# BlueFisher/Advanced-Soft-Actor-Critic

Measured on AMD Instinct MI355X. Metric: SAC train steps/sec (PER sample + grad step), batch 256, higher is better.
Workload: dtype f32; 1 GPU; cfg2: TEST vector obs(6) c_action(2) stock MLP, PER capacity 524288, n_step=4 V-trace; per_gpu_batch=256, global_batch=256, rows_resident=262144, replay_capacity=524288, n_step=4, burn_in_step=0, parallelism=single, ranks=1, hipgraph=True

## Files before the change

advanced-soft-actor-critic_amd/algorithm/fused_mlp.py:

```python
import weakref

import torch
from torch import nn

from asac_amd import native

from .nn_models.layers.linear_layers import LinearLayers, ResBlock
from .param_grads import (SUM_PARTIALS_LATER, DeferredPartialSums, direct_enabled, direct_param_grads,
                          direct_skips, flat_alias)

__all__ = ['StockMLP', 'describe_q', 'describe_policy', 'describe_dense', 'fused_dense', 'gauss_head']

MAX_WIDTH, MAX_HEAD = 64, 16
MAX_INPUT = 128
FUSED_DENSE = True


def _blocks_of(ll: LinearLayers):
    blocks, final = [], None
    for m in ll.dense:
        if isinstance(m, ResBlock):
            if final is not None or not isinstance(m.act, nn.GELU) or getattr(m.act, 'approximate', 'none') != 'none':
                return None
            blocks.append(m)
# ... 242 lines not shown
        x0, x1 = ctx.saved_tensors
        x1 = x1 if ctx.has_x1 else None
        need0, need1 = ctx.needs_input_grad[1], ctx.has_x1 and ctx.needs_input_grad[2]
        g0, g1, pg = _backward_delivering(ctx, x0, x1, grad_out, need0, need1)
        return (None, g0, g1, None, None, *pg)


class _MlpSelectFn(torch.autograd.Function):

    @staticmethod
    def forward(ctx, anchor, base, t, x1, mlp, param_grads, *params):
        x0 = base[:, t]
        out = mlp._launch_forward(x0, x1)
        ctx.mlp, ctx.param_grads, ctx.t, ctx.n_params = mlp, param_grads, t, len(params)
        ctx.save_for_backward(base, x1 if x1 is not None else base.new_empty(0))
        ctx.has_x1 = x1 is not None
        return out

    @staticmethod
    def backward(ctx, grad_out):
        base, x1 = ctx.saved_tensors
        x1 = x1 if ctx.has_x1 else None
        mlp, t = ctx.mlp, ctx.t
        need0, need1 = ctx.needs_input_grad[1], ctx.has_x1 and ctx.needs_input_grad[3]
        g0, g1, pg = _backward_delivering(ctx, base[:, t], x1, grad_out, need0, need1, reduce_members=False)
        g_base = None
        if g0 is not None:
            key = (tuple(base.shape), t % base.shape[1], base.device)
            g_base = mlp._window_grads.get(key)
            if g_base is None:
                if len(mlp._window_grads) > 4:
                    mlp._window_grads.clear()
                g_base = mlp._window_grads[key] = torch.zeros_like(base)
            torch.sum(g0, dim=0, out=g_base[:, t])
        if g1 is not None and x1.dim() == 2:
            g1 = g1.sum(0) if mlp.E > 1 else g1[0]
        return (None, g_base, None, g1, None, None, *pg)


class StockMLP:

    def __init__(self, desc, flat, grad_flat, start, member_stride, E, device, param_tensors=()):
        self.desc, self.E, self.member_stride = desc, E, member_stride
        self._window_grads = {}
        self.wide = desc.in0 + desc.in1 > MAX_WIDTH
        self.param_tensors = list(param_tensors)
        self.params = flat[start:start + E * member_stride]
        self.grad_params = None if grad_flat is None else grad_flat[start:start + E * member_stride]
        self.in0, self.in1 = desc.in0, desc.in1
        self.out_cols = desc.head_cols[0] + desc.head_cols[1]
        self._anchor = torch.zeros(1, device=device, requires_grad=True)
        self.accumulate = True
        self._workspace = None
        self._start, self._deferred_rows = start, None
        self.device = device

    @staticmethod
    def _rows(x, width):
        assert x.shape[-1] == width
        if x.dim() == 2 and x.stride(-1) == 1:
            return x
        return x.reshape(-1, width) if x.is_contiguous() else x.contiguous().view(-1, width)

    @staticmethod
    def _rows_in_place(x, width):
        assert x.shape[-1] == width
        if x.dim() == 3 and not x.is_contiguous() and x.stride(2) == 1 and x.stride(0) != x.stride(1) * x.shape[1]:
            return native.WindowRows(x)
        return StockMLP._rows(x, width)

    def _launch_forward(self, x0, x1, out=None):
        job, out = self.job(x0, x1, out)
        if isinstance(x0, native.WindowRows):
            native.mlp_forward_multi([job])
        else:
            native.mlp_forward(job)
        return out

    def _workspace_for(self, N):
        need = native.mlp_backward_workspace(self.member_stride, self.E, N)
        if self._workspace is None or self._workspace.numel() < need:
            self._workspace = torch.zeros(need, dtype=torch.float32, device=self.device)
        return self._workspace

    def _reduce_mode(self, defer):
        if defer:
            return native.MLP_REDUCE_DEFER
        return native.MLP_REDUCE_ACCUMULATE if self.accumulate else native.MLP_REDUCE_OVERWRITE

    def backward_qloss(self, x0, x1, target_q, y, weights, clip_eps, loss_out, defer=False, state_grads=False):
        N = x0.shape[-2]
        g0 = torch.empty((self.E, N, self.in0), dtype=torch.float32, device=self.device) if state_grads else None
        native.mlp_backward_qloss(self._pass(x0, x1), target_q, y, weights, clip_eps, loss_out, self.grad_params,
                                  self._workspace_for(N), self._reduce_mode(defer), grad_x0=g0)
        self._deferred_rows = N if defer else None
        return g0

    def backward_qloss_return_ok(self, N: int, ret) -> bool:
        return native.mlp_backward_qloss_return_ok(self._pass(None, None, N=N), ret)

    def backward_qloss_return(self, x0, x1, target_q, ret, weights, clip_eps, loss_out, defer=False, state_grads=False):
        N = x0.shape[-2]
        g0 = torch.empty((self.E, N, self.in0), dtype=torch.float32, device=self.device) if state_grads else None
        native.mlp_backward_qloss_return(self._pass(x0, x1), target_q, ret, weights, clip_eps, loss_out, self.grad_params,
                                         self._workspace_for(N), self._reduce_mode(defer), grad_x0=g0)
        self._deferred_rows = N if defer else None
        return g0

    def backward_policy_q(self, x0, x1, q_table, subset, E_sample):
        N = x0.shape[-2]
        g1 = torch.empty((self.E, N, self.in1), dtype=torch.float32, device=self.device)
        native.mlp_backward_policy_q(self._pass(x0, x1), q_table, subset, E_sample, g1)
        return g1

    def backward_policy_sample(self, x0, eps, grad_a, log_alpha, defer=False, offline=None):
        N = x0.shape[-2]
        native.mlp_backward_policy_sample(self._pass(x0, None), eps, grad_a, log_alpha, self.grad_params,
                                          self._workspace_for(N), self._reduce_mode(defer), offline=offline)
        self._deferred_rows = N if defer else None

    def policy_step_fused_ok(self, critics: 'StockMLP', N: int) -> bool:
        return (self.E == 1 and critics.E >= 2 and self.grad_params is not None and
                native.policy_step_fused_ok(critics.desc, critics.params, critics.member_stride, self.desc, self.params,
                                            self.member_stride, N))

    def policy_step_fused(self, critics: 'StockMLP', x0, action, eps, log_alpha, q_out=None, defer=False, subset=None,
                          sample_out=None, offline=None):
        N = x0.shape[-2]
        assert subset is not None or critics.E == 2
        a_out, logp_out, ls_out = sample_out if action is None else (None, None, None)
        native.policy_step_fused(critics.desc, critics.params, critics.member_stride, self.desc, self.params,
                                 self.member_stride, x0, N, action, eps, log_alpha, q_out, self.grad_params,
                                 self._workspace_for(N), self._reduce_mode(defer), subset=subset, a_out=a_out,
                                 logp_out=logp_out, ls_out=ls_out, offline=offline)
        self._deferred_rows = N if defer else None

    def adam_partials(self, opt, loss_out=None):
        N = self._deferred_rows
        assert N is not None, 'no deferred backward pending'
        tiles = native.mlp_backward_tiles(N, self.E)
        s0 = self._start
        s1 = s0 + self.E * self.member_stride
        native.adam_step_partials(self.params, self.grad_params, opt.exp_avg[s0:s1], opt.exp_avg_sq[s0:s1], opt.lr,
                                  opt.betas[0], opt.betas[1], opt.eps, opt.steps_done, self._workspace, tiles,
                                  self.E, self.member_stride, native.mlp_param_extent(self.desc),
                                  self.accumulate, loss_out, N if loss_out is not None else 0)
        self._deferred_rows = None

    def _pass(self, x0, x1, out=None, N=None) -> 'native.MlpJob':
        if N is None:
            N = x0.shape[0] if isinstance(x0, native.WindowRows) else x0.shape[-2]
        return native.mlp_job(self.desc, self.params, self.member_stride, self.E, x0, x1, N, out)

    def job(self, x0, x1, out=None):
        N = x0.shape[0] if isinstance(x0, native.WindowRows) else x0.shape[-2]
        if self.wide and isinstance(x0, native.WindowRows):
            x0 = x0.t.reshape(N, x0.t.shape[-1])
        if out is None:
            out = torch.empty((self.E, N, self.out_cols), dtype=torch.float32, device=self.device)
        assert out.shape == (self.E, N, self.out_cols) and out.is_contiguous()
        return self._pass(x0, x1, out), out

    def _launch_backward(self, x0, x1, grad_out, need0, need1, param_grads, reduce_members=True, defer=False,
                         grad_target=None, later=None):
        N = x0.shape[-2]
        E = self.E
        g0 = torch.empty((E, N, self.in0), dtype=torch.float32, device=self.device) if need0 else None
        g1 = torch.empty((E, N, self.in1), dtype=torch.float32, device=self.device) if need1 else None
        gp = ws = None
        mode = self._reduce_mode(defer and param_grads)
        if param_grads:
            gp = self.grad_params
            self._deferred_rows = N if defer else None
            if grad_target is not None:
                assert not defer
                gp, mode = grad_target, native.MLP_REDUCE_OVERWRITE
            if later is None or defer:
                ws = self._workspace_for(N)
            if later is not None and not defer:
                ws = torch.empty(native.mlp_backward_workspace(self.member_stride, E, N), dtype=torch.float32,
                                 device=self.device)
                tiles, used = native.mlp_backward_tiles(N, E), native.mlp_param_extent(self.desc)
                for e in range(E):
                    later.add(ws[e * self.member_stride:], tiles, 16 if tiles >= 64 else 1, E * self.member_stride, used,
                              gp[e * self.member_stride:], accumulate=mode == native.MLP_REDUCE_ACCUMULATE)
                mode = native.MLP_REDUCE_DEFER
        native.mlp_backward(self._pass(x0, x1), grad_out, g0, g1, gp, ws, reduce_mode=mode)
# ... 46 lines not shown
```

advanced-soft-actor-critic_amd/algorithm/sac_base.py:

```python
import contextlib
import logging
import random
from collections import defaultdict, namedtuple
from pathlib import Path

import numpy as np
import torch
from torch import distributions, nn
from torch.nn import functional

from asac_amd import native

from . import fused_gru, fused_linear
from .fused import DeviceNoise, FlatAdam, FlatParamGroup, squash_sample, squash_sample_ls, time_slice
from .fused_mlp import StockMLP, describe_policy, describe_q
from .nn_models import *
from .nn_models.layers.seq_layers import step_mask_cache
from .nn_models.representation import ModelSimpleRep
from .normalizer import Normalizer, fused_normalizer_applies
from .param_grads import direct_param_grads, learner_backward
from .batch_buffer import BatchBuffer
from .captured_step import CapturedStep
from .replay_buffer import PrioritizedReplayBuffer
from .sac_aux import AuxHeadsMixin
# ... 201 lines not shown
        self.ensemble_q_sample = ensemble_q_sample
        self.burn_in_step = burn_in_step
        self.n_step = n_step
        self.seq_encoder = seq_encoder
        self.write_summary_per_step = int(write_summary_per_step)
        self.save_model_per_step = int(save_model_per_step)
        self.batch_size = batch_size
        self.tau = tau
        self.update_target_per_step = update_target_per_step
        self.use_auto_alpha = use_auto_alpha
        self.target_d_alpha = target_d_alpha
        self.target_c_alpha = target_c_alpha
        self.d_policy_entropy_penalty = d_policy_entropy_penalty
        self.learning_rate = learning_rate
        self.gamma = gamma
        self.v_lambda = v_lambda
        self.v_rho = v_rho
        self.v_c = v_c
        self.clip_epsilon = clip_epsilon
        self.discrete_dqn_like = discrete_dqn_like
        self.discrete_dqn_epsilon = discrete_dqn_epsilon
        self.use_n_step_is = use_n_step_is
        self.siamese = siamese
        self.siamese_use_q = siamese_use_q
        self.siamese_use_adaptive = siamese_use_adaptive
        self.use_prediction = use_prediction
        self.transition_kl = transition_kl
        self.use_extra_data = use_extra_data
        self.curiosity = curiosity
        self.curiosity_strength = curiosity_strength
        self.use_rnd = use_rnd
        self.rnd_n_sample = rnd_n_sample
        self.use_normalization = use_normalization
        self.offline_enabled = offline_enabled
        self.offline_loss = offline_loss
        self.action_noise = action_noise

        hip_config = dict(hip_config or {})
        self._use_graph = bool(hip_config.get('use_graph', True))
        self._graph_warmup = int(hip_config.get('graph_warmup', 3))
        self._direct_graph_launch = bool(hip_config.get('direct_graph_launch', True))
        self._dist = hip_config.get('dist')
        self._use_fused_mlp = bool(hip_config.get('fused_mlp', True))
        self._graph_collectives = bool(hip_config.get('graph_collectives', True))
        self._twin_rep = bool(hip_config.get('twin_rep', True))
        self._fuse_linear_tanh = bool(hip_config.get('fused_linear_tanh', True))
        self._use_sidecars = bool(hip_config.get('sidecars', True))
        self._defer_is_weights = bool(hip_config.get('defer_is_weights', True))
        self._fused_policy_step = bool(hip_config.get('fused_policy_step', True))
        self._fused_forward_chain = bool(hip_config.get('fused_forward_chain', True))
        self._fused_td_chain = bool(hip_config.get('fused_td_chain', True))
        self._fused_td_update = bool(hip_config.get('fused_td_update', True))
        self._fused_q_return = bool(hip_config.get('fused_q_return', True))
        self._fused_q_state_grads = bool(hip_config.get('fused_q_state_grads', True))
        self._gru_backward_at = bool(hip_config.get('gru_backward_at', True))
        self._adjacent_cat = bool(hip_config.get('adjacent_cat', True))
        self._fold_rep_q_adam = bool(hip_config.get('fold_rep_q_adam', True))
        self._rep_grad_one_position = bool(hip_config.get('rep_grad_one_position', True))
        self._deferred_cat = bool(hip_config.get('deferred_cat', True))
        self._rep_from_burn_in = bool(hip_config.get('rep_from_burn_in', True))
        self._fused_curiosity = bool(hip_config.get('fused_curiosity', True))
        self._fused_discrete = bool(hip_config.get('fused_discrete', True))
        self._fused_dqn = bool(hip_config.get('fused_dqn', True))
        self._fused_rnd = bool(hip_config.get('fused_rnd', True))
        self._fused_offline = bool(hip_config.get('fused_offline', True))
        self._rnd_stacks = None
        self._rnd_buffers = {}
        self._fused_rnd_discrete = bool(hip_config.get('fused_rnd_discrete', True))
        self._drnd_stacks = None
        self._drnd_buffers = {}
        self._fused_act = bool(hip_config.get('fused_act', True))
        self._fused_siamese = bool(hip_config.get('fused_siamese', False))
        self._fused_hybrid = bool(hip_config.get('fused_hybrid', False))
        self._fused_normalizer = bool(hip_config.get('fused_normalizer', False))
        self.normalizer = None
        self._siamese_ws = {}
        self._fused_rpm_loss = bool(hip_config.get('fused_rpm_loss', True))
        self._rpm_single_backward = bool(hip_config.get('rpm_single_backward', True))
        self._fused_gating = bool(hip_config.get('fused_gating', True))
        self._rpm_conv_one_launch = bool(hip_config.get('rpm_conv_one_launch', True))
        self._lookahead = int(hip_config.get('lookahead', 0))
        assert self._lookahead in (0, 1), 'hip_config lookahead: 0 (synchronous sampling) or 1 (one batch in flight)'
        self._la_gather_sidecar = bool(hip_config.get('lookahead_gather_sidecar', True)) and self._use_sidecars
        self._head_gather_sidecar = bool(hip_config.get('head_gather_sidecar', True)) and self._use_sidecars
        self._head_gather = None
        self._head_gather_w = False
        self._head_plan_cache = None
        self._la_gather = None
        self._fuse_prediction_dense = bool(hip_config.get('fuse_prediction_dense', True))
        self._fused_q_loss_with_aux = bool(hip_config.get('fused_q_loss_with_aux', True))
        self._head_sums_members = bool(hip_config.get('head_sums_members', True))
        self._rep_epilogue, self._rep_epilogue_hp = False, None
        self._cat_mode = None
        self._g_state_base = None
        self._dist_sampling = hip_config.get('dist_sampling', 'throughput')
        self._dist_ready = False
        assert self._dist_sampling in ('throughput', 'parity')

        self._set_logger()

        if not use_replay_buffer:
            if self._dist is not None:
                raise ValueError('use_replay_buffer=False (the episode batch queue) is single-GPU: a data-parallel '
                                 "context (hip_config['dist']) is not supported with it")
            if self._lookahead:
                self._logger.info("hip_config['lookahead'] does not apply without a replay buffer: forced to 0")
# ... 161 lines not shown
        self._fq = self._ftq = self._fpi = None
        if self._use_fused_mlp and self.c_action_size and not self.d_action_sizes:
            dq = [describe_q(q) for q in self.model_q_list + self.model_target_q_list]
            seg = self._params.segments
            stride = seg['q_0'][1] - seg['q_0'][0]
            consecutive = all(seg[f'q_{i}'][0] == seg['q_0'][0] + i * stride for i in range(self.ensemble_q_num))
            if all(d is not None for d in dq) and consecutive:
                tseg = self._target_params.segments
                self._fq = StockMLP(dq[0], self._params.flat, self._params.grad, seg['q_0'][0], stride,
                                    self.ensemble_q_num, dev, [p for q in self.model_q_list for p in q.parameters()])
                self._ftq = StockMLP(dq[0], self._target_params.flat, None, tseg['q_0'][0], stride,
                                     self.ensemble_q_num, dev)
            dp = describe_policy(self.model_policy)
            if dp is not None:
                self._fpi = StockMLP(dp, self._params.flat, self._params.grad, seg['policy'][0],
                                     seg['policy'][1] - seg['policy'][0], 1, dev, list(self.model_policy.parameters()))
        self._wide_critics = self._fq is not None and self._fq.wide
        if self._wide_critics:
            self._la_gather_sidecar = False
        self._logger.info(f'fused stock MLP path: Q={self._fq is not None} policy={self._fpi is not None}')
        stock_only = {f'q_{i}' for i in range(self.ensemble_q_num)} | {'policy', 'alpha'}
        self._grads_overwrite = (self._fq is not None and self._fpi is not None and not self.offline_enabled
                                 and all(stop == start or name in stock_only
                                         for name, (start, stop) in self._params.segments.items()))
        if self._grads_overwrite:
            self._fq.accumulate = self._fpi.accumulate = False

        n, A, E, Es = self.n_step, self.c_action_size, self.ensemble_q_num, self.ensemble_q_sample
        f32 = dict(dtype=torch.float32, device=dev)
        A1 = max(A, 1)
        sizes = [B * (n + 1) * A1, B * A1, B * A1, B * (n + 1) * A1]
        self._eps_all = torch.zeros(sum(sizes), **f32)
        o = np.cumsum([0] + sizes)
        self._eps_y = self._eps_all[o[0]:o[1]].view(B, n + 1, A1)
        self._eps_pi = self._eps_all[o[1]:o[2]].view(B, A1)
        self._eps_alpha = self._eps_all[o[2]:o[3]].view(B, A1)
        self._eps_td = self._eps_all[o[3]:o[4]].view(B, n + 1, A1)
        names = ('y_dn', 'y_dnext', 'y_cn', 'y_cnext', 'pi_d', 'pi_c', 'td_dn', 'td_dnext', 'td_cn', 'td_cnext')
        self._subsets_all = torch.arange(Es, dtype=torch.int32, device=dev).repeat(len(names), 1).contiguous()
        self._subsets = {k: self._subsets_all[i] for i, k in enumerate(names)}
        self._y_buf = torch.zeros(B, **f32)
        self._y_td_buf = torch.zeros(B, **f32)
        self._td_error = torch.zeros(B, **f32)
        self._stats = {k: torch.zeros((), **f32) for k in ('d_entropy', 'c_entropy', 'loss_curiosity', 'loss_policy')}
        self._loss_q_e = torch.zeros(E, **f32)
        self._stats['loss_q'] = self._loss_q_e[0]
        self._grad_q = torch.zeros(E, B, **f32)
        self._mse_big_ws = torch.zeros(native.mse_mean_grad_workspace(), **f32) if self.use_prediction else None
        self._grad_logp = torch.zeros(B, **f32)
        self._branches = native.branches(self.d_action_sizes) if self.d_action_sizes else None
        self._discrete_grads = {}
        self._hybrid_bufs = {}
        self._ls_y = None
        self._cq_buf, self._tq_buf, self._cq_td_buf = (torch.zeros(E, B, 1, **f32) for _ in range(3))
        self._pi_q, self._pi_stats_src = torch.zeros(E, B, 1, **f32), None
        self._pi_a, self._pi_logp, self._pi_sampled = torch.zeros(B, A1, **f32), torch.zeros(B, **f32), False
        self._rep_twin = None
        if self._twin_rep and type(self.model_rep) is not ModelSimpleRep:
            from .fused_gru import TwinPass
            self._rep_twin = TwinPass(self.model_rep, self.model_target_rep)

    def _build_ckpt(self) -> None:
        ck = self.ckpt_dict = {'global_step': self.global_step}
        if self.optimizer_rep is not None:
            ck['model_rep'], ck['model_target_rep'], ck['optimizer_rep'] = \
                self.model_rep, self.model_target_rep, self.optimizer_rep
        for i in range(self.ensemble_q_num):
            ck[f'model_q_{i}'] = self.model_q_list[i]
            ck[f'model_target_q_{i}'] = self.model_target_q_list[i]
            ck[f'optimizer_q_{i}'] = self.optimizer_q_list[i]
        ck['model_policy'], ck['optimizer_policy'] = self.model_policy, self.optimizer_policy
        ck['log_d_alpha'], ck['log_c_alpha'] = self.log_d_alpha, self.log_c_alpha
        if self.use_auto_alpha:
            ck['optimizer_alpha'] = self.optimizer_alpha
        if self.curiosity == CURIOSITY.FORWARD:
            ck['model_forward_dynamic'] = self.model_forward_dynamic
        elif self.curiosity == CURIOSITY.INVERSE:
            ck['model_inverse_dynamic'] = self.model_inverse_dynamic
        if self.curiosity is not None:
            ck['optimizer_curiosity'] = self.optimizer_curiosity
        self._aux_ckpt(ck)
        total = sum(p.numel() for m in ck.values() if isinstance(m, nn.Module) for p in m.parameters())
        self._logger.info(f'Parameters: {total}')

    def _init_or_restore(self, last_ckpt: int | None) -> None:
        self.ckpt_dir = None
        if not self.model_abs_dir:
            self._update_target_variables()
            return
        self.ckpt_dir = ckpt_dir = Path(self.model_abs_dir).joinpath('model')
        ckpts = sorted(int(p.stem) for p in ckpt_dir.glob('*.pth')) if ckpt_dir.exists() else []
        ckpt_dir.mkdir(parents=True, exist_ok=True)
        if not ckpts:
            self._logger.info('Initializing from scratch')
            self._update_target_variables()
            return
        if last_ckpt is None or last_ckpt not in ckpts:
            if last_ckpt is not None:
                self._logger.warning(f'{last_ckpt} NOT IN {ckpts}, using {ckpts[-1]}')
            last_ckpt = ckpts[-1]
        path = ckpt_dir.joinpath(f'{last_ckpt}.pth')
        restored = torch.load(path, map_location=self.device, weights_only=True)
        failed = False
        for name, obj in self.ckpt_dict.items():
            if name not in restored:
                self._logger.warning(f'{name} not in {last_ckpt}.pth')
# ... 761 lines not shown
            if d_q_online is not None:
                args.td_error_out = td_out.data_ptr()
            native.discrete_return(args, self._branches, [q[0] for q in nx_qs], d_logits, action=nx_actions,
                                   q_online=d_q_online)
            d_y = y_out.unsqueeze(-1)
        elif self.d_action_sizes:
            sub_next, sub_n = self._subsets[subset_prefix + '_dnext'], self._subsets[subset_prefix + '_dn']
            self.noise.subset_(sub_next, E)
            self.noise.subset_(sub_n, E)
            stacked = torch.stack([q[0] for q in nx_qs])
            mean_next = stacked[:, :, 1:].index_select(0, sub_next.long()).mean(0)
            mean_n = stacked[:, :, :-1].index_select(0, sub_n.long()).mean(0)
            probs = d_policy.probs
            n_p, next_p = probs[:, :-1], probs[:, 1:]
            d_alpha = torch.exp(self.log_d_alpha)
            v_n = torch.sum(n_p * (mean_n - d_alpha * torch.log(n_p.clamp(min=1e-8))), -1) / self.d_action_branch_size
            v_next = torch.sum(next_p * (mean_next - d_alpha * torch.log(next_p.clamp(min=1e-8))), -1) \
                / self.d_action_branch_size
            pi, mu = self._stored_action_ratios(d_policy, n_mu_probs, nx_actions) if self.use_n_step_is else (None, None)
            d_y = torch.empty(n_rewards.shape[0], dtype=torch.float32, device=self.device)
            args = self._vtrace_args(n_rewards, n_dones, n_last_masks, n_padding_masks, d_y)
            native.vtrace_return_direct(args, v_n.contiguous(), v_next.contiguous(), pi, mu)
            d_y = d_y.unsqueeze(-1)

        if self.c_action_size:
            sub_n, sub_next = self._subsets[subset_prefix + '_cn'], self._subsets[subset_prefix + '_cnext']
            self.noise.subset_(sub_n, E)
            self.noise.subset_(sub_next, E)
            if q_table is not None:
                q_tab = q_table
            elif nx_qs is not None:
                q_tab = torch.stack([q[1] for q in nx_qs]).squeeze(-1)
            else:
                q_tab = self._c_q_values(True, nx_states, a_tanh, nx_obses_list)
            ret = self._c_return(q_tab, logp, c_pi, n_mu_probs, sub_n, sub_next, n_rewards, n_dones, n_last_masks,
                                 n_padding_masks, y_out, q_online, td_out)
            if launch:
                self._launch_return(ret)
            c_y = y_out.unsqueeze(-1)
        return (d_y, c_y) if launch else (d_y, c_y, ret)

    def _stock_q_targets(self, job_tq, job_pi, ls, window, policy_sample):
        nx_states, nx_actions = window[3], window[4]
        ls = ls[0].view(*nx_states.shape[:2], 2 * self.c_action_size)
        pre = self._return_sample_epilogue([job_tq, job_pi], 1, ls, nx_actions, self._eps_y, policy_sample)
        if pre is None:
            native.mlp_forward_multi([job_tq, job_pi])
        sample, stored_pi = pre or (None, None)
        _, c_y, ret = self._get_y(*window, eps_buf=self._eps_y, subset_prefix='y', y_out=self._y_buf, ls=ls,
                                  sample=sample, stored_pi=stored_pi, policy_sample=policy_sample and pre is None,
                                  launch=False)
        return c_y, ret

    def _stock_q_backward(self, x0, a0, ret, c_y, priority_is, fold, fused_return, state_grads=False):
        w = priority_is.reshape(-1).contiguous() if priority_is is not None else None
        t_q = self._tq_buf.view(self.ensemble_q_num, -1)
        if fused_return and self._fq.backward_qloss_return_ok(x0.shape[-2], ret.args):
            g0 = self._fq.backward_qloss_return(x0, a0, t_q, ret.args, w, self.clip_epsilon, self._loss_q_e,
                                                defer=fold, state_grads=state_grads)
        else:
            self._launch_return(ret)
            g0 = self._fq.backward_qloss(x0, a0, t_q, c_y.reshape(-1), w, self.clip_epsilon, self._loss_q_e,
                                         defer=fold, state_grads=state_grads)
        if fold:
            self._fq.adam_partials(self.optimizer_q_list[0], loss_out=self._loss_q_e)
        return g0

    @torch.no_grad()
    def _train_rep_q_stock(self, n_last_masks, n_padding_masks, nx_obses_list, nx_states, nx_actions, n_rewards,
                           n_dones, n_mu_probs, priority_is, policy_sample):
        E, B = self.ensemble_q_num, nx_states.shape[0]
        x0 = StockMLP._rows(nx_states[:, 0], self.state_size)
        a0 = StockMLP._rows(nx_actions[:, 0], self.c_action_size)
        xs = StockMLP._rows(nx_states, self.state_size)
        job_tq, _ = self._ftq.job(x0, a0, out=self._tq_buf)
        job_pi, ls = self._fpi.job(xs, None)
        T, A = nx_states.shape[1], self.c_action_size
        window = (n_last_masks, n_padding_masks, nx_obses_list, nx_states, nx_actions, n_rewards, n_dones,
                  n_mu_probs if self.use_n_step_is else None)
        fused = None
        if self._fused_forward_chain and self.curiosity is None:
            f32 = dict(dtype=torch.float32, device=self.device)
            a_y, logp_y = torch.empty((B, T, A), **f32), torch.empty((B, T), **f32)
            c_pi = torch.empty((B, T, A), **f32) if self.use_n_step_is else None
            job_q, q_tab = self._ftq.job(xs, a_y.view(-1, A))
            fused = native.pi_q_job(job_pi, job_q, self._eps_y, a_y, logp_y, T,
                                    action=nx_actions if self.use_n_step_is else None,
                                    action_offset=self.d_action_summed_size, prob_out=c_pi,
                                    eps2=self._eps_pi if policy_sample else None, t2=0,
                                    a2_out=self._pi_a, logp2_out=self._pi_logp)
            if not native.policy_sample_q_forward_ok(fused):
                fused = None
        riders = None
        if fused is not None and self._head_gather is not None:
            ring = self._head_ring_job(fused, job_tq, self._head_gather, nx_states, nx_actions)
            if ring is not None:
                fused, riders = ring, [self._head_gather['sidecar_w' if self._head_gather_w else 'sidecar']]
                self._head_gather = None
        self._join_head_gather()
        if fused is not None:
            self.noise.normal_(self._eps_y)
            if policy_sample:
                self.noise.normal_(self._eps_pi)
                self._pi_sampled = True
            native.policy_sample_q_forward(fused, [job_tq], sidecars=riders if riders is not None else self._take_la_gather())
            _, c_y, ret = self._get_y(*window, eps_buf=self._eps_y, subset_prefix='y', y_out=self._y_buf,
                                      ls=ls[0].view(B, T, 2 * A), sample=(a_y, logp_y), stored_pi=c_pi,
                                      q_table=q_tab.view(E, B, T), launch=False)
        else:
            c_y, ret = self._stock_q_targets(job_tq, job_pi, ls, window, policy_sample)
        opt = self.optimizer_q_list[0]
        fold = self._dist is None and opt.start == self._fq._start and self._params.span('rep')[0] == self._params.span('rep')[1]
        self._stock_q_backward(x0, a0, ret, c_y, priority_is, fold, fused_return=fused is not None and self._fused_q_return)
        if not fold:
            self._finish_rep_q(None, None)

    def _head_ring_job(self, fused, job_tq, head, nx_states, nx_actions):
        rb, b = self.replay_buffer, self.burn_in_step
        obs, act = rb._batch[f'obs_{self.obs_names[0]}'], rb._batch['action']
        if b != rb.prev_n or nx_states.shape[1] + b != rb.window:
            return None
        for view, whole in ((nx_states, obs), (nx_actions, act)):
            at = whole[:, b:]
            if view.data_ptr() != at.data_ptr() or view.stride() != at.stride() or view.shape != at.shape:
                return None
        job = native.pi_q_ring_rows(fused, rb._ids, head['index_ring'], rb.capacity, rb.prev_n, rb.window, b, head['x0'],
                                    head['action'], x_j0=b, x_action_offset=self.d_action_summed_size)
        return job if native.policy_sample_q_forward_ok(job, [job_tq]) else None

    def _train_rep_q(self, n_last_masks, n_padding_masks, nx_obses_list, nx_states, nx_actions, n_rewards,
                     n_dones, n_mu_probs, priority_is, aux=None, policy_sample=False, state_base=None):
        if (self._stock_c_only() and aux is None and self.clip_epsilon > 0 and not nx_states.requires_grad
                and self.optimizer_rep is None):
            return self._train_rep_q_stock(n_last_masks, n_padding_masks, nx_obses_list, nx_states, nx_actions,
                                           n_rewards, n_dones, n_mu_probs, priority_is, policy_sample)
        self._join_head_gather()
        dsum = self.d_action_summed_size
        obs_list = [o[:, 0] for o in nx_obses_list]
        state, action = nx_states[:, 0], nx_actions[:, 0]
        if state_base is not None and not nx_states.requires_grad:
            state = state_base[0][:, state_base[1]]
        d_action, c_action = action[..., :dsum], action[..., dsum:]

        if (self._fused_q_state_grads and self._fq is not None and self._ftq is not None and self._fpi is not None
                and not self.d_action_sizes
                and self.c_action_size and self.clip_epsilon > 0 and aux is None and state_base is not None
                and state_base[0].dim() == 3 and state.requires_grad):
            base, t = state_base
            with torch.no_grad():
                x0 = StockMLP._rows(base.detach()[:, t], self.state_size)
                a0 = StockMLP._rows(c_action, self.c_action_size)
                states_y = nx_states.detach()
                job_tq, _ = self._ftq.job(x0, a0, out=self._tq_buf)
                job_pi, ls_y = self._fpi.job(StockMLP._rows_in_place(states_y, self.state_size), None)
                c_y, ret = self._stock_q_targets(
                    job_tq, job_pi, ls_y, (n_last_masks, n_padding_masks, nx_obses_list, states_y, nx_actions, n_rewards,
                                           n_dones, n_mu_probs if self.use_n_step_is else None), policy_sample)
                fold = self._dist is None and self._fold_rep_q_adam and self._rep_q_adam_alike()
                g0 = self._stock_q_backward(x0, a0, ret, c_y, priority_is, fold, fused_return=self._fused_q_return,
                                            state_grads=True)
                g_base = self._g_state_base
                if g_base is None or g_base.shape != base.shape:
                    g_base = self._g_state_base = torch.zeros_like(base)
                at_position = self._gru_backward_at and fused_gru.is_fused_top(base)
                from_head = not at_position and self._head_sums_members and fused_linear.is_fused_head_output(base)
                if not (at_position or from_head):
# ... 110 lines not shown
    def _finish_rep_q(self, total_loss, loss_q0, aux=None, ctx=None):
        if total_loss is not None:
            with learner_backward():
                total_loss.backward(retain_graph=aux is not None and self.use_prediction)
            self._stats['loss_q'].copy_(loss_q0.detach())
        start, stop = self._params.span('rep', f'q_{self.ensemble_q_num - 1}')
        if aux is None:
            if self._dist is not None:
                self._dist.all_reduce_grads(self._params.grad, start, stop)
            self.optimizer_q_list[0].step(start, stop)
            return
        grads_rep_main = [p.grad.detach() for p in self.model_rep.parameters()]
        grads_q_main = [[p.grad.detach() for p in q.parameters()] for q in self.model_q_list]
        if self.siamese is not None:
            n_obs = [o[:, :-1] for o in ctx['nx_obses_list']]
            self._train_siamese_representation_learning(grads_rep_main, grads_q_main, aux['n_indexes'],
                                                        ctx['n_padding_masks'], n_obs, aux['n_pre_actions'],
                                                        aux['n_pre_seq_hidden_states'])
        q_start = self._params.span('q_0')[0]
        if self._dist is not None:
            self._dist.all_reduce_grads(self._params.grad, q_start, stop)
        self.optimizer_q_list[0].step(q_start, stop)
        if self.use_prediction:
            self._train_rpm(grads_rep_main, ctx['nx_obses_list'], ctx['nx_states'], aux['nx_target_states'],
                            ctx['nx_actions'][:, :-1], ctx['n_rewards'])
        if self.optimizer_rep is not None:
            if self._dist is not None:
                self._dist.all_reduce_grads(self._params.grad, *self._params.span('rep'))
            self.optimizer_rep.step()

    def _stock_c_only(self) -> bool:
        return (self._fpi is not None and self._fq is not None and bool(self.c_action_size)
                and not self.d_action_sizes and (not (self.offline_enabled and self.offline_loss) or self._offline_fused()))

    def _offline_fused(self) -> bool:
        return fused_offline_applies(
            enabled=self._fused_offline, plain_learner=type(self)._plain_learner,
            offline_loss=self.offline_enabled and self.offline_loss, c_action_size=self.c_action_size,
            d_action_sizes=self.d_action_sizes, stock_networks=self._fq is not None and self._fpi is not None,
            data_parallel=self._dist is not None,
            float32_on_device=self._params.flat.dtype == torch.float32 and self._params.flat.is_cuda)

    def _offline_plain(self) -> bool:
        return bool(self._fused_offline and type(self)._plain_learner and self._dist is None
                    and self._params.flat.dtype == torch.float32 and self._params.flat.is_cuda)

    @torch.no_grad()
    def _train_policy_stock(self, state, ls=None, offline=None):
        A, E = self.c_action_size, self.ensemble_q_num
        x = StockMLP._rows(state, self.state_size)
        B = x.shape[0]
        fusable = (self._fused_policy_step and self.ensemble_q_sample == 2 and self._fpi.policy_step_fused_ok(self._fq, B))
        sample_out = None
        if ls is None and not self._pi_sampled and fusable:
            f32 = dict(dtype=torch.float32, device=self.device)
            self.noise.normal_(self._eps_pi)
            sample_out = (torch.empty((B, A), **f32), torch.empty(B, **f32), torch.empty((B, 2 * A), **f32))
            a_tanh, logp, scale = sample_out[0], sample_out[1], sample_out[2][:, A:]
        else:
            if ls is None:
                ls = self._fpi._launch_forward(x, None)[0]
            loc, scale = ls[..., :A], ls[..., A:]
            if self._pi_sampled:
                a_tanh, logp, self._pi_sampled = self._pi_a, self._pi_logp, False
            else:
                self.noise.normal_(self._eps_pi)
                a_tanh = torch.empty((B, A), dtype=torch.float32, device=self.device)
                logp = torch.empty(B, dtype=torch.float32, device=self.device)
                native.squash_sample_fwd(loc, scale, self._eps_pi, a_tanh, logp)
        sub = self._subsets['pi_c']
        self.noise.subset_(sub, E)
        self._pi_stats_src = (logp, scale) if offline is None else (
            logp, scale, sample_out[2] if sample_out is not None else ls, self._eps_pi, offline)
        opt = self.optimizer_policy
        fold = self._dist is None and (opt.start, opt.stop) == (self._fpi._start, self._fpi._start + self._fpi.member_stride)
        if fusable and a_tanh.is_contiguous():
            self._fpi.policy_step_fused(self._fq, x, None if sample_out is not None else a_tanh, self._eps_pi,
                                        self.log_c_alpha, q_out=self._pi_q, defer=fold, subset=sub if E != 2 else None,
                                        sample_out=sample_out, offline=offline)
        else:
            c_qs = self._fq._launch_forward(x, a_tanh, out=self._pi_q)
            g_a = self._fq.backward_policy_q(x, a_tanh, c_qs.view(E, B), sub if self.ensemble_q_sample != E else None,
                                             self.ensemble_q_sample)
            self._fpi.backward_policy_sample(x, self._eps_pi, g_a, self.log_c_alpha, defer=fold, offline=offline)
        if fold:
            self._fpi.adam_partials(opt)
            return
        if self._dist is not None:
            self._dist.all_reduce_grads(self._params.grad, *self._params.span('policy'))
        opt.step()

    def _train_policy(self, obs_list, state, action, mu_d_policy_probs, ls=None):
        dsum, E = self.d_action_summed_size, self.ensemble_q_num
        offline = self.offline_enabled and self.offline_loss
        if self._stock_c_only():
            return self._train_policy_stock(state, ls, offline=action[..., dsum:] if offline else None)
        if self._discrete_fused(state.shape[0]):
            logits = self._discrete_logits(state, obs_list)
            with torch.no_grad():
                d_qs = [q(state, action[..., dsum:], obs_list)[0] for q in self.model_q_list]
            sub = self._subsets['pi_d']
            self.noise.subset_(sub, E)
            _, grad_logits = self._discrete_grad_buffers(state.shape[0])
            native.discrete_policy_loss_grad(self._branches, logits.detach(), d_qs, sub, self.ensemble_q_sample,
                                             mu_d_policy_probs, self.log_d_alpha, self.d_policy_entropy_penalty,
                                             self._stats['loss_policy'], grad_logits, self._stats['d_entropy'])
            pi_inputs = list(self.model_policy.parameters())
            with direct_param_grads(only=pi_inputs):
                torch.autograd.backward([logits], [grad_logits], inputs=pi_inputs)
            self.optimizer_policy.step()
            return
        if self._hybrid_fused(state.shape[0]):
            logits, loc, scale = self._hybrid_heads(state, obs_list)
            with torch.no_grad():
                d_qs = [q(state, action[..., dsum:], obs_list)[0] for q in self.model_q_list]
            sub_d = self._subsets['pi_d']
            self.noise.subset_(sub_d, E)
            self.noise.normal_(self._eps_pi)
            a_tanh, logp = squash_sample(loc, scale, self._eps_pi)
            c_qs = torch.stack([q(state, a_tanh, obs_list)[1] for q in self.model_q_list]).squeeze(-1)
            sub_c = self._subsets['pi_c']
            self.noise.subset_(sub_c, E)
            buf = self._hybrid_buffers(state.shape[0])
            native.hybrid_policy_loss_grad(
                self._branches, logits.detach(), d_qs, sub_d, mu_d_policy_probs, self.log_d_alpha,
                self.d_policy_entropy_penalty, logp.detach(), c_qs.detach().contiguous(),
                sub_c if self.ensemble_q_sample != E else None, self.ensemble_q_sample, self.log_c_alpha, scale.detach(),
                self._stats['loss_policy'], buf['grad_logits'], buf['grad_logp'], buf['grad_cq'], self._stats['d_entropy'],
                self._stats['c_entropy'])
# ... 860 lines not shown
```

advanced-soft-actor-critic_amd/csrc/mlp.hip:

```cpp
#include "asac_common.h"
#include "asac_gelu.h"
#include "asac_sidecar.h"
#include "asac_squash.h"
#include "asac_vtrace.h"

#include <cmath>

namespace asac {

constexpr int kP = 66;
constexpr int kMaxW = 64;
constexpr int kMaxB = ASAC_MLP_MAX_BLOCKS;
constexpr int kHeadPad = 16;
#ifndef ASAC_PS_WAVES
#define ASAC_PS_WAVES 16
#endif
#ifndef ASAC_PIQ_WAVES
#define ASAC_PIQ_WAVES 8
#endif
constexpr int kPiQThreads = 64 * ASAC_PIQ_WAVES;
template <int TM> constexpr int threads_of() { return TM * 16; }

inline int mlp_tile_rows(int64_t N, int E) { return ((N + 15) / 16) * (int64_t)(E > 0 ? E : 1) <= 256 ? 16 : 32; }

using f32x4 = __attribute__((ext_vector_type(4))) float;

#ifdef ASAC_MLP_STAMPS
__device__ unsigned long long g_mlp_stamps[32];
#define MLP_STAMP(i)                                                                             \
    do {                                                                                         \
        if (blockIdx.x == 0 && blockIdx.y == 0 && threadIdx.x == 0) g_mlp_stamps[i] = wall_clock64(); \
    } while (0)
#define MLP_STAMP_AT(i, t)                                                                       \
    do {                                                                                         \
        if (blockIdx.x == 0 && blockIdx.y == 0 && threadIdx.x == (t)) g_mlp_stamps[i] = wall_clock64(); \
    } while (0)
#else
#define MLP_STAMP(i)
#define MLP_STAMP_AT(i, t)
#endif

__device__ __forceinline__ void lds_barrier() {
    __builtin_amdgcn_fence(__ATOMIC_RELEASE, "workgroup", "local");
    __builtin_amdgcn_s_barrier();
    __builtin_amdgcn_fence(__ATOMIC_ACQUIRE, "workgroup", "local");
}

__device__ __forceinline__ void loads_landed() { __builtin_amdgcn_s_waitcnt(0x0F70); }

__device__ __forceinline__ int round4(int v) { return (v + 3) & ~3; }

template <int THREADS>
__device__ __forceinline__ void stage_matrix(float* dst, const float* __restrict__ src, int rows, int cols) {
    if (rows == kMaxW && cols == kMaxW && (reinterpret_cast<uintptr_t>(src) & 15) == 0) {
        constexpr int U = 1024 / THREADS;
        const float4* s4 = reinterpret_cast<const float4*>(src);
        float4 v[U];
#pragma unroll
        for (int u = 0; u < U; ++u) v[u] = s4[threadIdx.x + u * THREADS];
// ... 779 lines not shown
    s += __shfl_xor(s, 16, 64);
    s += __shfl_xor(s, 32, 64);
    if (lane < 16 && c < J) out[c] = s;
}

__device__ __forceinline__ void grad_weight_tiles(const float* __restrict__ delta, int jbase, const float* __restrict__ xprev,
                                                  int J, int K, float* __restrict__ out, int worker, int workers) {
    if (worker < 0) return;
    const int lane = threadIdx.x & 63;
    const int lr = lane & 15, lk = lane >> 4;
    const int njt = (J + 15) >> 4, nkt = (K + 15) >> 4;
    const bool vec = (K & 3) == 0 && (reinterpret_cast<uintptr_t>(out) & 15) == 0;
    for (int t = worker; t < njt * nkt; t += workers) {
        const int jt = t / nkt, kt = t - jt * nkt;
        float dv[4], xv[4];
#pragma unroll
        for (int i = 0; i < 4; ++i) {
            dv[i] = delta[(4 * i + lk) * kP + jbase + jt * 16 + lr];
            xv[i] = xprev[(4 * i + lk) * kP + kt * 16 + lr];
        }
        __builtin_amdgcn_sched_barrier(0);
        f32x4 acc0 = {0.f, 0.f, 0.f, 0.f}, acc1 = {0.f, 0.f, 0.f, 0.f};
        acc0 = __builtin_amdgcn_mfma_f32_16x16x4f32(xv[0], dv[0], acc0, 0, 0, 0);
        acc1 = __builtin_amdgcn_mfma_f32_16x16x4f32(xv[1], dv[1], acc1, 0, 0, 0);
        acc0 = __builtin_amdgcn_mfma_f32_16x16x4f32(xv[2], dv[2], acc0, 0, 0, 0);
        acc1 = __builtin_amdgcn_mfma_f32_16x16x4f32(xv[3], dv[3], acc1, 0, 0, 0);
        const f32x4 acc = acc0 + acc1;
        const int j = jt * 16 + lr, k0 = kt * 16 + 4 * lk;
        if (j >= J) continue;
        float* o = out + j * K + k0;
        if (vec && k0 + 3 < K) {
            *reinterpret_cast<float4*>(o) = make_float4(acc[0], acc[1], acc[2], acc[3]);
        } else {
#pragma unroll
            for (int r = 0; r < 4; ++r)
                if (k0 + r < K) o[r] = acc[r];
        }
    }
}
template <int NW = ASAC_PS_WAVES>
__device__ __forceinline__ void ps_grad_weight(const float* __restrict__ delta, int jbase, const float* __restrict__ xprev,
                                               int J, int K, float* __restrict__ out, int first_wave = 0) {
    grad_weight_tiles(delta, jbase, xprev, J, K, out, ((threadIdx.x >> 6) + NW - first_wave) & (NW - 1), NW);
}

template <bool RET>
struct RetIn {};
template <>
struct RetIn<true> {
    asac_vtrace_args_t v;
    int32_t seg;
};

template <int TM, bool WIDE, int NB, bool RET = false, int W8 = 0>
__global__ __launch_bounds__(W8 ? 64 * W8 : TM * 16) void k_mlp_bwd(const MlpArgs a, const RetIn<RET> rv) {
    static_assert(W8 == 0 || ((W8 == 8 || W8 == 16) && TM == 16 && NB == 3 && !WIDE), "8 / 16 waves: 16-row tiles of the stock networks");
    constexpr int THREADS = W8 ? 64 * W8 : threads_of<TM>();
    constexpr int RT = TM / 16;
    constexpr bool fixed = NB > 0;
    static_assert(!(fixed && WIDE), "the fixed-shape path has a first layer of <= 64 inputs");
    extern __shared__ __attribute__((aligned(16))) unsigned char smem_raw[];
    MlpBwdLds<TM>& L = *reinterpret_cast<MlpBwdLds<TM>*>(smem_raw);
    const int e = blockIdx.y;
    const int64_t row0 = (int64_t)blockIdx.x * TM;
    const float* P = a.params + e * a.member_stride;
    float* part = a.partial ? a.partial + ((int64_t)blockIdx.x * gridDim.y + e) * a.member_stride : nullptr;
    const int wave = threadIdx.x >> 6, lane = threadIdx.x & 63;
    const bool comp = !W8 || wave < 4;
    const int rt = wave % RT, ct = comp ? wave / RT : 0;
    const int nb = fixed ? NB : a.d.n_blocks;
    const int K0 = a.d.in0 + a.d.in1;
    const int O = a.d.head_cols[0] + a.d.head_cols[1];
    const int col = ct * 16 + (lane & 15);

    MLP_STAMP(0);
    [[maybe_unused]] float ql_tq[4] = {0.f, 0.f, 0.f, 0.f}, ql_w[4] = {1.f, 1.f, 1.f, 1.f}, ql_y[4] = {0.f, 0.f, 0.f, 0.f};
    constexpr bool wide = WIDE;
    float* x_hi = L.x[kMaxB];
    float* w_hi = L.w[nb < kMaxB ? nb : kMaxB - 1];
    if constexpr (fixed) {
        const StageScalars q = stage_scalars<NB>(a, e);
        constexpr int SLOTS = TM * 64 / THREADS;
        float in_lo[SLOTS];
        fetch_input_tile_fixed<THREADS, false, SLOTS>(q, e, row0, in_lo);
        const int r = threadIdx.x >> 4, c = threadIdx.x & 15;
        const int64_t row = row0 + r;
        float gin = 0.f;
        if (a.gout && r < TM) {
            const float t = a.gout[((int64_t)e * a.N + (row < a.N ? row : a.N - 1)) * O + (c < O ? c : O - 1)];
            gin = (row < a.N && c < O) ? t : 0.f;
        }
        StagedNet<THREADS> regs;
        net_fetch_fixed<THREADS, NB>(q, regs);
        if constexpr (W8 != 0) {
            if (!a.gout && !a.eps && !a.q_table && wave < RT) {
#pragma unroll
                for (int rr = 0; rr < 4; ++rr) {
                    const int64_t lr_row = row0 + wave * 16 + 4 * (lane >> 4) + rr;
                    const int64_t rc = lr_row < a.N ? lr_row : a.N - 1;
                    ql_tq[rr] = a.tq[(int64_t)e * a.N + rc];
                    if (a.w) ql_w[rr] = a.w[rc];
                    if constexpr (!RET) ql_y[rr] = a.y[rc];
                }
            }
        }
        if constexpr (RET) {
            const asac_vtrace_args_t& v = rv.v;
            const int n = v.n, pitch = (n + 1) | 1;
            float* s_d = reinterpret_cast<float*>(smem_raw + sizeof(MlpBwdLds<TM>));
            float* s_c = s_d + TM * pitch;
            float* s_v0 = s_c + TM * pitch;
            const int f = threadIdx.x, fr = f / n, ft = f - fr * n;
            const bool have = f < TM * n && row0 + fr < a.N;
            VtraceStepRaw raw{};
// ... 267 lines not shown
    if (comp && (a.gx0 || a.gx1)) {
#pragma unroll
        for (int r = 0; r < 4; ++r) {
            const int64_t row = row0 + rt * 16 + 4 * (lane >> 4) + r;
            if (row >= a.N) continue;
            if (col < a.d.in0) {
                if (a.gx0) a.gx0[((int64_t)e * a.N + row) * a.d.in0 + col] = g[r];
            } else if (col < K0) {
                if (a.gx1) a.gx1[((int64_t)e * a.N + row) * a.d.in1 + (col - a.d.in0)] = g[r];
            }
            const int ch = col + kMaxW;
            if (wide && ch < K0) {
                if (ch < a.d.in0) {
                    if (a.gx0) a.gx0[((int64_t)e * a.N + row) * a.d.in0 + ch] = g_hi[r];
                } else if (a.gx1) {
                    a.gx1[((int64_t)e * a.N + row) * a.d.in1 + (ch - a.d.in0)] = g_hi[r];
                }
            }
        }
    }
    MLP_STAMP(10);
}

constexpr int kPsWaves = ASAC_PS_WAVES;
constexpr int kPsThreads = 64 * kPsWaves;
constexpr int kPsSlots = 1024 / kPsThreads;
constexpr int kPsRows = 16;

struct PsQLds {
    float w[3][kMaxW * kP];
    float head[kHeadPad * kP];
    float bias[3][kMaxW];
    float head_bias[kHeadPad];
    float xs[2][kPsRows * kP];
};
struct PsPiLds {
    float w[3][kMaxW * kP];
    float head[kHeadPad * kP];
    float bias[3][kMaxW];
    float head_bias[kHeadPad];
    float x[4][kPsRows * kP];
    float delta[kPsRows * kP];
    float delta2[kPsRows * kP];
};
struct PsLds {
    PsQLds q[2];
    float ga[2][kPsRows * kHeadPad];
    float qv[2][kPsRows];
    float ls[kPsRows * 2 * kHeadPad];
    float act[kPsRows * kHeadPad];
};
static_assert(sizeof(PsPiLds) <= 2 * sizeof(PsQLds), "the policy phase reuses the critics' LDS");

struct PolicyStepArgs {
    MlpArgs q, pi;
    float* q_out;
    float* a_out;
    float* logp_out;
    float* ls_out;
};

__device__ __forceinline__ void ps_fetch_tile(const StageScalars& q, int64_t row0, float (&v)[kPsSlots]) {
    const int in0 = q.in0, in1 = q.in1;
    const rsrc_t r0 = make_rsrc(q.x0);
    const rsrc_t r1 = make_rsrc(q.x1, in1 > 0 ? 0x7fffffffu : 0u);
#pragma unroll
    for (int u = 0; u < kPsSlots; ++u) {
        const int i = threadIdx.x + u * kPsThreads;
        const int r = i >> 6, c = i & 63;
        const uint32_t row = (uint32_t)row0 + (uint32_t)r;
        const bool live = (int64_t)row0 + r < q.N;
        const unsigned o0 = (live && c < in0) ? (row * (uint32_t)q.x0_rs + (uint32_t)c) * 4u : kOob;
        const unsigned o1 = (live && c >= in0 && c < in0 + in1) ? (row * (uint32_t)q.x1_rs + (uint32_t)(c - in0)) * 4u : kOob;
        v[u] = __builtin_bit_cast(float, buf_ld(r0, o0) | buf_ld(r1, o1));
    }
}
__device__ __forceinline__ void ps_put_tile(const float (&v)[kPsSlots], float* xs) {
#pragma unroll
    for (int u = 0; u < kPsSlots; ++u) {
        const int i = threadIdx.x + u * kPsThreads;
        xs[(i >> 6) * kP + (i & 63)] = v[u];
    }
}

template <bool OFFLINE>
__global__ __launch_bounds__(kPsThreads) void k_policy_step(const PolicyStepArgs a_by_value) {
    extern __shared__ __attribute__((aligned(16))) unsigned char smem_raw[];
    const ASAC_KARG PolicyStepArgs& a = *static_cast<const ASAC_KARG PolicyStepArgs*>(kernarg_base());
    PsLds& L = *reinterpret_cast<PsLds*>(smem_raw);
    PsPiLds& P = *reinterpret_cast<PsPiLds*>(smem_raw);
    const int wave = threadIdx.x >> 6, lane = threadIdx.x & 63;
    const int m = wave >> 2, ct = wave & 3;
    const int col = ct * 16 + (lane & 15);
    const int64_t row0 = (int64_t)blockIdx.x * kPsRows;
    const int64_t N = a.pi.N;
    const int A = a.pi.d.head_cols[0];
    const int S = a.q.d.in0, K0q = a.q.d.in0 + a.q.d.in1, K0p = a.pi.d.in0;
    MLP_STAMP(0);

    const int e0 = a.q.subset ? a.q.subset[0] : 0, e1 = a.q.subset ? a.q.subset[1] : 1;
    const StageScalars s0 = stage_scalars<3>(a.q, e0), s1 = stage_scalars<3>(a.q, e1), sp = stage_scalars<3>(a.pi, 0);
    const bool sample_here = a.q.x1 == nullptr;
    float in_q[kPsSlots] = {}, in_pi[kPsSlots];
    if (!sample_here) ps_fetch_tile(s0, row0, in_q);
    ps_fetch_tile(sp, row0, in_pi);
    StagedNet<kPsThreads> r0, r1, rp;
    net_fetch_fixed<kPsThreads, 3>(s0, r0);
    net_fetch_fixed<kPsThreads, 3>(s1, r1);
    net_fetch_fixed<kPsThreads, 3>(sp, rp);
    float ev = 0.f, gl = 0.f;
    {
        const int lrow = threadIdx.x / (A > 0 ? A : 1), d = threadIdx.x - lrow * A;
        if ((int)threadIdx.x < kPsRows * A && row0 + lrow < N) ev = a.pi.eps[(row0 + lrow) * A + d];
        gl = expf(*a.pi.log_alpha) * (1.f / (float)N);
    }
    [[maybe_unused]] float av = 0.f;
    if constexpr (OFFLINE) {
        const int lrow = threadIdx.x / (A > 0 ? A : 1), d = threadIdx.x - lrow * A;
        if ((int)threadIdx.x < kPsRows * A && row0 + lrow < N) av = a.pi.off_action[(row0 + lrow) * a.pi.off_row_stride + d];
    }
    if (sample_here) {
        net_put_fixed<kPsThreads, 3>(rp, P);
        ps_put_tile(in_pi, P.x[0]);
        __syncthreads();
#pragma unroll
        for (int l = 0; l < 3; ++l) {
            if (wave < 4) {
                const float* xin = P.x[l & 1];
                float* xout = P.x[(l & 1) ^ 1];
                const f32x4 acc = l > 0 ? gemm_tile(xin, P.w[l], kMaxW, 0, wave) : gemm_tile(xin, P.w[l], round4(K0p), 0, wave);
                const int pc = wave * 16 + (lane & 15);
                const float bias = P.bias[l][pc];
                const bool res = a.pi.d.residual[l] != 0;
                f32x2_g ya, yb, unused;
                gelu_parts2((f32x2_g){acc[0] + bias, acc[1] + bias}, ya, unused);
                gelu_parts2((f32x2_g){acc[2] + bias, acc[3] + bias}, yb, unused);
                const float yv[4] = {ya.x, ya.y, yb.x, yb.y};
#pragma unroll
                for (int r = 0; r < 4; ++r) {
                    const int row = 4 * (lane >> 4) + r;
                    float y = yv[r];
                    if (res) y += xin[row * kP + pc];
                    xout[row * kP + pc] = y;
                }
            }
            __syncthreads();
        }
        if (wave < 4) {
            const f32x4 acc = gemm_tile(P.x[1], P.head, kMaxW, 0, 0);
            const int hc = lane & 15;
            const float mine = wave == 0 ? acc[0] : wave == 1 ? acc[1] : wave == 2 ? acc[2] : acc[3];
            const int lrow = 4 * (lane >> 4) + wave;
            const float v = head_value(a.pi.d, hc, mine + P.head_bias[hc]);
            L.ls[lrow * 2 * kHeadPad + hc] = v;
            if (a.ls_out && row0 + lrow < N && hc < 2 * A) a.ls_out[(row0 + lrow) * (2 * A) + hc] = v;
        }
        __syncthreads();
        if (threadIdx.x < kPsRows) {
            const int lrow = threadIdx.x;
            const int64_t r = row0 + lrow;
            float* arow = L.act + lrow * kHeadPad;
            if (r < N) {
                float lp;
                squash_sample_at(L.ls + lrow * 2 * kHeadPad, L.ls + lrow * 2 * kHeadPad + A, a.pi.eps + r * A, A, arow, &lp, nullptr);
                for (int d = 0; d < A; ++d) a.a_out[r * A + d] = arow[d];
                a.logp_out[r] = lp;
            } else {
                for (int d = 0; d < A; ++d) arow[d] = 0.f;
            }
        }
        __syncthreads();
        ps_put_tile(in_pi, L.q[0].xs[0]);
        ps_put_tile(in_pi, L.q[1].xs[0]);
    } else {
        ps_put_tile(in_q, L.q[0].xs[0]);
        ps_put_tile(in_q, L.q[1].xs[0]);
    }
    net_put_fixed<kPsThreads, 3>(r0, L.q[0]);
    net_put_fixed<kPsThreads, 3>(r1, L.q[1]);
    __syncthreads();
    if (sample_here) {
        if ((int)threadIdx.x < kPsRows * A) {
            const int lrow = threadIdx.x / A, d = threadIdx.x - lrow * A;
            const float v = L.act[lrow * kHeadPad + d];
            L.q[0].xs[0][lrow * kP + S + d] = v;
            L.q[1].xs[0][lrow * kP + S + d] = v;
        }
        __syncthreads();
    }
    MLP_STAMP(1);

    const bool qwave = wave < 8;
    PsQLds& Q = L.q[qwave ? m : 0];
    f32x4 z[3];
    int cur = 0;
#pragma unroll
    for (int l = 0; l < 3; ++l) {
        if (qwave) {
        const float* xin = Q.xs[cur];
        float* xout = Q.xs[cur ^ 1];
        const f32x4 acc = l > 0 ? gemm_tile(xin, Q.w[l], kMaxW, 0, ct) : gemm_tile(xin, Q.w[l], round4(K0q), 0, ct);
        const float bias = Q.bias[l][col];
        const bool res = a.q.d.residual[l] != 0;
        f32x2_g ya, yb, da, db;
        gelu_parts2((f32x2_g){acc[0] + bias, acc[1] + bias}, ya, da);
        gelu_parts2((f32x2_g){acc[2] + bias, acc[3] + bias}, yb, db);
        const float yv[4] = {ya.x, ya.y, yb.x, yb.y};
        z[l] = f32x4{da.x, da.y, db.x, db.y};
#pragma unroll
        for (int r = 0; r < 4; ++r) {
            const int row = 4 * (lane >> 4) + r;
            float y = yv[r];
            if (res) y += xin[row * kP + col];
            xout[row * kP + col] = y;
        }
        }
        __syncthreads();
        cur ^= 1;
    }
    MLP_STAMP(2);
    if (qwave && ct == 0) {
        const f32x4 raw = gemm_tile(Q.xs[cur], Q.head, kMaxW, 0, 0);
        if ((lane & 15) == 0) {
#pragma unroll
            for (int r = 0; r < 4; ++r) {
                const int lrow = 4 * (lane >> 4) + r;
                const float qv = raw[r] + Q.head_bias[0];
                L.qv[m][lrow] = qv;
                if (a.q_out && row0 + lrow < N) a.q_out[(int64_t)(m ? e1 : e0) * N + row0 + lrow] = qv;
            }
        }
    }
    __syncthreads();
    MLP_STAMP(3);
    float* qdelta = Q.xs[cur ^ 1];
    if (qwave) {
        const int t = threadIdx.x & 255;
        const int r = t >> 4, c = t & 15;
        float g = 0.f;
        if (c == 0 && row0 + r < N) {
            const int best = L.qv[1][r] < L.qv[0][r] ? 1 : 0;
            if (best == m) g = -1.f / (float)N;
        }
        qdelta[r * kP + c] = g;
    }
    __syncthreads();
    MLP_STAMP(4);
    f32x4 g = {0.f, 0.f, 0.f, 0.f};
    if (qwave) g = gemm_tile_nt(qdelta, Q.head, kHeadPad, 0, ct);
#pragma unroll
    for (int l = 2; l >= 0; --l) {
        qdelta = Q.xs[cur ^ (l & 1)];
        if (qwave) {
#pragma unroll
            for (int r = 0; r < 4; ++r) qdelta[(4 * (lane >> 4) + r) * kP + col] = g[r] * z[l][r];
        }
        __syncthreads();
        if (qwave && (l > 0 || (ct * 16 < K0q && ct * 16 + 16 > S))) {
            f32x4 gin = gemm_tile_nt(qdelta, Q.w[l], kMaxW, 0, ct);
            if (a.q.d.residual[l]) gin += g;
            g = gin;
        }
    }
    if (qwave && col >= S && col < K0q) {
#pragma unroll
        for (int r = 0; r < 4; ++r) L.ga[m][(4 * (lane >> 4) + r) * kHeadPad + (col - S)] = g[r];
    }
    __syncthreads();
    MLP_STAMP(5);

    net_put_fixed<kPsThreads, 3>(rp, P);
    ps_put_tile(in_pi, P.x[0]);
    if (threadIdx.x < kPsRows * kHeadPad) P.delta[(threadIdx.x >> 4) * kP + (threadIdx.x & 15)] = 0.f;
    loads_landed();
    __syncthreads();
    MLP_STAMP(6);
    f32x4 zp[3];
#pragma unroll
    for (int l = 0; l < 3; ++l) {
        if (wave < 4) {
            const float* xin = P.x[l];
            float* xout = P.x[l + 1];
            const f32x4 acc = l > 0 ? gemm_tile(xin, P.w[l], kMaxW, 0, wave) : gemm_tile(xin, P.w[l], round4(K0p), 0, wave);
            const int pc = wave * 16 + (lane & 15);
            const float bias = P.bias[l][pc];
            const bool res = a.pi.d.residual[l] != 0;
            f32x2_g ya, yb, da, db;
            gelu_parts2((f32x2_g){acc[0] + bias, acc[1] + bias}, ya, da);
            gelu_parts2((f32x2_g){acc[2] + bias, acc[3] + bias}, yb, db);
            const float yv[4] = {ya.x, ya.y, yb.x, yb.y};
            zp[l] = f32x4{da.x, da.y, db.x, db.y};
#pragma unroll
            for (int r = 0; r < 4; ++r) {
                const int row = 4 * (lane >> 4) + r;
                float y = yv[r];
                if (res) y += xin[row * kP + pc];
                xout[row * kP + pc] = y;
            }
        }
        __syncthreads();
    }
    MLP_STAMP(7);
    if (wave == 0) {
        const f32x4 raw = gemm_tile(P.x[3], P.head, kMaxW, 0, 0);
        const int hc = lane & 15;
#pragma unroll
        for (int r = 0; r < 4; ++r) P.delta[(4 * (lane >> 4) + r) * kP + hc] = raw[r] + P.head_bias[hc];
    }
    __syncthreads();
    MLP_STAMP(8);
    if ((int)threadIdx.x < kPsRows * A) {
        const int lrow = threadIdx.x / A, d = threadIdx.x - lrow * A;
        const int64_t row = row0 + lrow;
        float g_loc = 0.f, g_scale = 0.f;
        const float raw_l = P.delta[lrow * kP + d], raw_s = P.delta[lrow * kP + A + d];
        if (row < N) {
            const float loc = head_value(a.pi.d, d, raw_l), sc = head_value(a.pi.d, A + d, raw_s);
            const float u = loc + ev * sc;
            const float t = tanhf(u);
            const float one_m = 1.f - t * t;
            float ga = 0.f;
            ga += L.ga[0][lrow * kHeadPad + d];
            ga += L.ga[1][lrow * kHeadPad + d];
            float gx = ga * one_m;
            if (one_m > 1e-2f) gx += gl * ((float)A * 2.f * t);
            if constexpr (OFFLINE) gx += offline_grad_u(u, av, 1.f / (float)N);
            g_loc = gx * head_deriv(a.pi.d, d, raw_l);
            g_scale = (gx * ev - gl / sc) * head_deriv(a.pi.d, A + d, raw_s);
        }
        P.delta[lrow * kP + d] = g_loc;
        P.delta[lrow * kP + A + d] = g_scale;
    }
    __syncthreads();
    MLP_STAMP(9);
    float* part = a.pi.partial + (int64_t)blockIdx.x * a.pi.member_stride;
    ps_grad_weight(P.delta, 0, P.x[3], A, kMaxW, part + a.pi.d.head_w_off[0]);
    ps_grad_weight(P.delta, A, P.x[3], A, kMaxW, part + a.pi.d.head_w_off[1], 4);
    if (wave == 7) {
        const int c = lane & 15, rq = (lane >> 4) * 4;
        float sb = 0.f;
#pragma unroll
        for (int r = 0; r < 4; ++r) sb += P.delta[(rq + r) * kP + c];
        sb += __shfl_xor(sb, 16, 64);
        sb += __shfl_xor(sb, 32, 64);
        if (lane < 16) {
            if (c < A) part[a.pi.d.head_b_off[0] + c] = sb;
            else if (c < 2 * A) part[a.pi.d.head_b_off[1] + c - A] = sb;
        }
    }
    f32x4 gp = {0.f, 0.f, 0.f, 0.f};
    if (wave < 4) gp = gemm_tile_nt(P.delta, P.head, kHeadPad, 0, wave);
    MLP_STAMP(10);
#pragma unroll
    for (int l = 2; l >= 0; --l) {
        const int Kin = l == 0 ? K0p : kMaxW;
        float* pdelta = (l & 1) ? P.delta : P.delta2;
        if (wave < 4) {
            const int pc = wave * 16 + (lane & 15);
#pragma unroll
            for (int r = 0; r < 4; ++r) pdelta[(4 * (lane >> 4) + r) * kP + pc] = gp[r] * zp[l][r];
        }
        __syncthreads();
        ps_grad_weight(pdelta, 0, P.x[l], kMaxW, Kin, part + a.pi.d.w_off[l]);
        grad_bias<kPsRows>(pdelta, 0, kMaxW, part + a.pi.d.b_off[l]);
        if (l > 0 && wave < 4) {
            f32x4 gin = gemm_tile_nt(pdelta, P.w[l], kMaxW, 0, wave);
            if (a.pi.d.residual[l]) gin += gp;
            gp = gin;
        }
        MLP_STAMP(11 + (2 - l));
    }
}

struct StockJobArg {
    const float *P, *x0, *x1;
    float* out;
    int32_t member_stride, N, x0_rs, x0_ms, x1_rs, x1_ms, x0_sb, x0_T;
    int32_t in0, in1, h0, h1, hw0, hw1, hb0, hb1;
    int32_t w_off[3], b_off[3];
    int32_t residual_bits, head_transform;
};
static_assert(sizeof(StockJobArg) == 128, "StockJobArg");

template <typename JOB>
__device__ __forceinline__ MlpFwdArgs expand_stock(const JOB& j) {
    MlpFwdArgs a;
    a.d.in0 = j.in0, a.d.in1 = j.in1, a.d.n_blocks = 3;
#pragma unroll
    for (int l = 0; l < kMaxB; ++l) {
        a.d.width[l] = l < 3 ? kMaxW : 0;
        a.d.residual[l] = l < 3 ? (j.residual_bits >> l) & 1 : 0;
        a.d.w_off[l] = l < 3 ? j.w_off[l] : 0;
        a.d.b_off[l] = l < 3 ? j.b_off[l] : 0;
    }
    a.d.head_cols[0] = j.h0, a.d.head_cols[1] = j.h1;
    a.d.head_w_off[0] = j.hw0, a.d.head_w_off[1] = j.hw1;
    a.d.head_b_off[0] = j.hb0, a.d.head_b_off[1] = j.hb1;
    a.d.head_transform = j.head_transform, a.d.reserved_ = 0;
    a.params = j.P, a.member_stride = j.member_stride;
    a.x0 = j.x0, a.x0_rs = j.x0_rs, a.x0_ms = j.x0_ms;
    a.x1 = j.x1, a.x1_rs = j.x1_rs, a.x1_ms = j.x1_ms;
    a.x0_sb = j.x0_sb, a.x0_T = j.x0_T, a.pad_ = 0;
    a.N = j.N, a.out = j.out;
    return a;
}

struct PiQLds {
    float head[kHeadPad * kP];
    float bias[kMaxB][kMaxW];
    float head_bias[kHeadPad];
    float xs[2][16 * kP];
    float w[3][kMaxW * kP];
    float qw[3][kMaxW * kP];
    float qhead[kHeadPad * kP];
    float qbias[3][kMaxW];
    float qhead_bias[kHeadPad];
// ... 8 lines not shown
    float (&bias)[3][kMaxW];
    float (&head_bias)[kHeadPad];
};

struct StoredProbArg {
    const float* action;
    float* out;
    int32_t T, a_sb, a_st, a_off, p_sb, p_st, p_off, pad_;
};
struct PiQLaunch {
    StockJobArg pi, q;
    const float *eps, *eps2;
    float *a_out, *logp_out, *a2_out, *logp2_out;
    StoredProbArg sp;
    int32_t E, tile_groups, blocks, T, t2;
    int32_t x_n, x_blocks;
    int32_t x_E[ASAC_MLP_MAX_JOBS], x_first_block[ASAC_MLP_MAX_JOBS], x_tile_stride[ASAC_MLP_MAX_JOBS];
    StockJobArg x_job[ASAC_MLP_MAX_JOBS];
};


__device__ __forceinline__ StageScalars stage_scalars_stock(const ASAC_KARG StockJobArg& j, int e) {
    StageScalars q;
    q.P = j.P + e * j.member_stride;
    q.x0 = j.x0, q.x1 = j.in1 > 0 ? j.x1 : j.x0;
    q.N = j.N, q.x0_rs = j.x0_rs, q.x0_ms = j.x0_ms, q.x1_rs = j.x1_rs, q.x1_ms = j.x1_ms, q.x0_sb = j.x0_sb;
    q.in0 = j.in0, q.in1 = j.in1, q.x0_T = j.x0_T;
    q.h0 = j.h0, q.h1 = j.h1;
    q.hw0 = j.hw0, q.hw1 = j.hw1, q.hb0 = j.hb0, q.hb1 = j.hb1;
#pragma unroll
    for (int l = 0; l < 3; ++l) q.w_off[l] = j.w_off[l], q.b_off[l] = j.b_off[l];
    ASAC_PIN(q.P); ASAC_PIN(q.x0); ASAC_PIN(q.x1);
    ASAC_PIN(q.N); ASAC_PIN(q.x0_rs); ASAC_PIN(q.x0_ms); ASAC_PIN(q.x1_rs); ASAC_PIN(q.x1_ms); ASAC_PIN(q.x0_sb);
    ASAC_PIN(q.in0); ASAC_PIN(q.in1); ASAC_PIN(q.x0_T); ASAC_PIN(q.h0); ASAC_PIN(q.h1);
    ASAC_PIN(q.hw0); ASAC_PIN(q.hw1); ASAC_PIN(q.hb0); ASAC_PIN(q.hb1);
#pragma unroll
    for (int l = 0; l < 3; ++l) { ASAC_PIN(q.w_off[l]); ASAC_PIN(q.b_off[l]); }
    return q;
}

__device__ __forceinline__ StageScalars stage_scalars_stock_like(const ASAC_KARG StockJobArg& j, int e, const StageScalars& rows) {
    StageScalars q = rows;
    q.P = j.P + e * j.member_stride;
    q.in1 = j.in1;
    q.h0 = j.h0, q.h1 = j.h1;
    q.hw0 = j.hw0, q.hw1 = j.hw1, q.hb0 = j.hb0, q.hb1 = j.hb1;
#pragma unroll
    for (int l = 0; l < 3; ++l) q.w_off[l] = j.w_off[l], q.b_off[l] = j.b_off[l];
    ASAC_PIN(q.P); ASAC_PIN(q.in1); ASAC_PIN(q.h0); ASAC_PIN(q.h1);
    ASAC_PIN(q.hw0); ASAC_PIN(q.hw1); ASAC_PIN(q.hb0); ASAC_PIN(q.hb1);
#pragma unroll
    for (int l = 0; l < 3; ++l) { ASAC_PIN(q.w_off[l]); ASAC_PIN(q.b_off[l]); }
    return q;
}

template <bool WINDOW, bool RING = false, bool SINGLE = false>
__device__ __forceinline__ void pi_q_tiles(const ASAC_KARG PiQLaunch& a, PiQLds& L, const ASAC_KARG RingArg* ring = nullptr) {
    static_assert(!(RING && WINDOW), "ring-addressed rows have their own (sample, row) addressing");
    constexpr int THREADS = kPiQThreads;
    constexpr int SLOTS = 1024 / kPiQThreads;
    const bool comp = (threadIdx.x >> 6) < 4;
    const int e = (int)blockIdx.x % a.E, group = (int)blockIdx.x / a.E;
    const int wave = threadIdx.x >> 6, lane = threadIdx.x & 63;
    const int col = wave * 16 + (lane & 15);
    const int A = a.pi.h0, S = a.q.in0;
    const int K0p = a.pi.in0, K0q = a.q.in0 + a.q.in1;
    const int N = a.pi.N;
    const int n_tiles = (int)((N + 15) / 16);
    const bool writer = e == 0;
    MLP_STAMP(0);

    const StageScalars sp = stage_scalars_stock(a.pi, 0);
    const StageScalars sq = stage_scalars_stock_like(a.q, e, sp);
    float in_lo[SLOTS];
    int64_t id_lo[SLOTS];
    RingStage R{};
    if constexpr (RING) {
        R = ring_stage<false>(*ring, ring->j0, a.T, 0);
        ring_tile_ids<THREADS, SLOTS>(sp, R, (int64_t)group * 16, id_lo);
    } else {
        fetch_input_tile_fixed<THREADS, WINDOW, SLOTS>(sp, 0, (int64_t)group * 16, in_lo);
    }
    float ev_pre[2];
    {
        const float* e1 = a.eps;
#pragma unroll
        for (int h = 0; h < 2; ++h) ev_pre[h] = e1[min(group * 16 * A + lane + 64 * h, N * A - 1)];
    }
    StagedNet<THREADS> rp, rq;
    net_fetch_fixed<THREADS, 3>(sp, rp);
    net_fetch_fixed<THREADS, 3>(sq, rq);
    if constexpr (RING) ring_tile_rows<THREADS, SLOTS, false>(sp, R, (int64_t)group * 16, id_lo, in_lo);
    put_input_tile<THREADS, SLOTS>(in_lo, L.xs[0]);
    net_put_fixed<THREADS, 3>(rp, L);
    PiQCritic C{L.qw, L.qhead, L.qbias, L.qhead_bias};
    __syncthreads();
    MLP_STAMP(1);

    constexpr bool single = SINGLE;
    float av_pre[2] = {0.f, 0.f}, ev2_pre[2] = {0.f, 0.f};
    if (single) net_put_fixed<THREADS, 3>(rq, C);

    for (int tile = group; tile < n_tiles; tile += a.tile_groups) {
        const int row0 = tile * 16;
        if (!single && tile != group) {
            if constexpr (RING) {
// ... 521 lines not shown
    if (stock3(*desc, a.params, a.member_stride) && offsets32(a))
        return launch(k_mlp_fwd<TM, false, 3>, sizeof(MlpLds<TM>), attr_stock);
    return launch(k_mlp_fwd<TM, false, 0>, sizeof(MlpLds<TM>), attr_done);
}

template <int TM, int NB>
static int launch_forward_multi(const asac_mlp_job_t* jobs, int n_jobs, const SidecarsDev& sc, hipStream_t s,
                                const SampleEpis* epis = nullptr) {
    static bool attr_done = false, attr_done_epi = false;
    if (int rc = epis ? set_lds_limit(reinterpret_cast<const void*>(k_mlp_fwd_multi_sampled<TM, NB>), sizeof(MlpLds<TM>),
                                      attr_done_epi, "asac_mlp_forward_multi_sampled: hipFuncSetAttribute")
                      : set_lds_limit(reinterpret_cast<const void*>(k_mlp_fwd_multi<TM, NB>), sizeof(MlpLds<TM>), attr_done,
                                      "asac_mlp_forward_multi: hipFuncSetAttribute"))
        return rc;
    MlpMultiArgs m{};
    m.n = n_jobs;
    int blocks = 0;
    size_t lds = 0;
    for (int k = 0; k < n_jobs; ++k) {
        const size_t need = mlp_fwd_lds_bytes(jobs[k].desc->n_blocks, false, TM);
        lds = need > lds ? need : lds;
    }
    const int per_cu = lds <= 80 * 1024 ? 2 : 1;
    for (int k = 0; k < n_jobs; ++k) {
        const asac_mlp_job_t& j = jobs[k];
        m.job[k] = make_args(j);
        m.job[k].x0_T = j.x0_window_T;
        m.job[k].x0_sb = j.x0_sample_stride;
        m.job[k].out = j.out;
        m.E[k] = j.E;
        m.first_block[k] = blocks;
        m.tile_stride[k] = mlp_tile_groups(j.N, j.E, per_cu, TM);
        blocks += m.tile_stride[k] * j.E;
    }
    m.blocks = blocks;
    const SidecarsDev none{};
    for (int rep = 0; rep < g_launch_repeat; ++rep) {
        const bool last = rep == g_launch_repeat - 1;
        if (epis)
            hipLaunchKernelGGL((k_mlp_fwd_multi_sampled<TM, NB>), dim3((unsigned)(blocks + (last ? sc.blocks : 0))),
                               dim3(threads_of<TM>()), lds, s, m, *epis, last ? sc : none);
        else
            hipLaunchKernelGGL((k_mlp_fwd_multi<TM, NB>), dim3((unsigned)(blocks + (last ? sc.blocks : 0))),
                               dim3(threads_of<TM>()), lds, s, m, last ? sc : none);
    }
    return finish_launch(epis ? "asac_mlp_forward_multi_sampled" : "asac_mlp_forward_multi");
}

#ifndef ASAC_BWD_WAVES
#define ASAC_BWD_WAVES 16
#endif
template <int TM>
static int launch_backward(const char* where, const asac_mlp_desc_t* desc, MlpArgs& a, int E, int tiles, hipStream_t s,
                           const RetIn<true>* ret = nullptr) {
    static bool attr_done = false, attr_wide = false, attr_stock = false, attr_ret = false;
    const bool wide = wide_input(*desc);
    const bool stock = !wide && stock3(*desc, a.params, a.member_stride) && offsets32(a);
    constexpr int w8 = TM == 16 ? ASAC_BWD_WAVES : 0;
    constexpr int stock_threads = w8 ? 64 * w8 : threads_of<TM>();
    auto launch = [&](auto kernel, bool& attr, size_t lds_limit, int threads, size_t lds,
                      const auto& ret_in) -> int {
        if (int rc = set_lds_limit(reinterpret_cast<const void*>(kernel), lds_limit, attr, where)) return rc;
        ASAC_LAUNCH(kernel, dim3(tiles, E), dim3(threads), lds, s, a, ret_in);
        return 0;
    };
    const size_t lds = sizeof(MlpBwdLds<TM>);
    constexpr size_t spare = w8 ? (size_t)TM * kP * sizeof(float) : 0;
    if (ret) {
        const size_t lds_ret = lds + (size_t)(2 * ((ret->v.n + 1) | 1) + 2) * TM * sizeof(float) + spare;
        if (!stock || TM * ret->v.n > stock_threads || lds_ret > 128 * 1024) return bad_arg(where);
        return launch(k_mlp_bwd<TM, false, 3, true, w8>, attr_ret, 128 * 1024, stock_threads, lds_ret, *ret);
    }
    if (wide) return launch(k_mlp_bwd<TM, true, 0>, attr_wide, lds, threads_of<TM>(), lds, RetIn<false>{});
    if (stock) return launch(k_mlp_bwd<TM, false, 3, false, w8>, attr_stock, lds + spare, stock_threads, lds + spare, RetIn<false>{});
    return launch(k_mlp_bwd<TM, false, 0>, attr_done, lds, threads_of<TM>(), lds, RetIn<false>{});
}

static void reduce_partials(const asac_mlp_desc_t* desc, const float* workspace, int tiles, int E, int64_t member_stride,
                            float* grad, int reduce_mode, const float* loss_partial, float* loss_out, float inv_n,
                            hipStream_t s) {
    const int64_t used = asac_mlp_param_extent(desc);
    const int accumulate = reduce_mode == ASAC_MLP_REDUCE_ACCUMULATE ? 1 : 0;
    if (tiles >= kSlicedFrom)
        hipLaunchKernelGGL(k_mlp_reduce_partials_sliced, dim3((unsigned)((used + 63) / 64), (unsigned)E),
                           dim3(64 * kReduceSlices), 0, s, workspace, tiles, E, member_stride, used, grad, accumulate,
                           loss_partial, loss_out, inv_n);
    else
        hipLaunchKernelGGL(k_mlp_reduce_partials, dim3((unsigned)((used + 255) / 256), (unsigned)E), dim3(256), 0, s,
                           workspace, tiles, E, member_stride, used, grad, accumulate, loss_partial, loss_out, inv_n);
}

static int mlp_backward_common(const char* where, const asac_mlp_job_t& j, MlpArgs& a, float* grad_params, float* workspace,
                               int reduce_mode, float* loss_out, hipStream_t s, const RetIn<true>* ret = nullptr) {
    const int tiles = (int)asac_mlp_backward_tiles(j.N, j.E);
    a.partial = grad_params ? workspace : nullptr;
    a.loss_partial = workspace ? workspace + (int64_t)tiles * j.E * j.member_stride : nullptr;
    if (int rc = mlp_tile_rows(j.N, j.E) == 16 ? launch_backward<16>(where, j.desc, a, j.E, tiles, s, ret)
                                               : launch_backward<32>(where, j.desc, a, j.E, tiles, s, ret))
        return rc;
    if (grad_params && reduce_mode != ASAC_MLP_REDUCE_DEFER)
        reduce_partials(j.desc, workspace, tiles, j.E, j.member_stride, grad_params, reduce_mode,
                        loss_out ? a.loss_partial : nullptr, loss_out, 1.f / (float)j.N, s);
    return finish_launch(where);
}

extern "C" {

int asac_mlp_forward(const asac_mlp_job_t* job, void* stream) {
    if (!job || !job_ok(*job, true) || job->x0_window_T != 0) return bad_arg("asac_mlp_forward");
    MlpArgs a = make_args(*job);
    a.out = job->out;
    return mlp_tile_rows(job->N, job->E) == 16 ? launch_forward<16>(job->desc, a, job->E, job->N, as_stream(stream))
                                               : launch_forward<32>(job->desc, a, job->E, job->N, as_stream(stream));
}

static bool sample_epilogue_ok(const asac_mlp_job_t& j, const asac_mlp_sample_epilogue_t& h) {
    const asac_squash_job_t& q = h.sample;
    if (!j.desc || !gauss_head(*j.desc) || j.E != 1) return false;
    const int A = j.desc->head_cols[0];
    if (A < 1 || 2 * A > 16 || q.A != A || q.rows != j.N || j.N * (int64_t)A >= 0x7fffffffLL) return false;
    if (!q.eps && !q.action && !h.eps2) return false;
    if (q.eps && (!q.a_tanh_out || !q.logp_out)) return false;
    if (q.x_out) return false;
    if ((q.action || h.eps2) && (q.T <= 0 || j.N % q.T != 0)) return false;
    if (q.action) {
        const int64_t sb = j.N / q.T;
        if (!q.prob_out || sb * q.action_stride_b + (int64_t)q.T * q.action_stride_t + q.action_offset + A >= 0x7fffffffLL ||
            sb * q.prob_stride_b + (int64_t)q.T * q.prob_stride_t + q.prob_offset + A >= 0x7fffffffLL ||
            q.action_stride_b < 0 || q.action_stride_t < 0 || q.prob_stride_b < 0 || q.prob_stride_t < 0)
            return false;
    }
    if (h.eps2 && (!h.a2_out || !h.logp2_out || h.t2 < 0 || h.t2 >= q.T)) return false;
    return true;
}

static SampleEpis sample_epis(const asac_mlp_sample_epilogue_t* epilogues, int n_jobs) {
    SampleEpis epis{};
    for (int k = 0; k < n_jobs; ++k) {
        const asac_mlp_sample_epilogue_t& h = epilogues[k];
        const asac_squash_job_t& q = h.sample;
        SampleEpi& d = epis.e[k];
        d.on = (q.eps || q.action || h.eps2) ? 1 : 0;
        if (!d.on) continue;
        d.eps = q.eps, d.eps2 = h.eps2, d.a_out = q.a_tanh_out, d.logp_out = q.logp_out, d.a2_out = h.a2_out, d.logp2_out = h.logp2_out;
        d.action = q.action, d.prob_out = q.prob_out;
        d.a_sb = (int32_t)q.action_stride_b, d.a_st = (int32_t)q.action_stride_t, d.a_off = q.action_offset;
        d.p_sb = (int32_t)q.prob_stride_b, d.p_st = (int32_t)q.prob_stride_t, d.p_off = q.prob_offset;
        d.A = q.A, d.T = q.T > 0 ? q.T : 1, d.t2 = h.t2;
    }
    return epis;
}

static int forward_multi(const asac_mlp_job_t* jobs, int n_jobs, const SampleEpis* epis, const asac_sidecar_t* sidecars_host,
                         int n_sidecars, void* stream) {
    SidecarsDev sc{};
// ... 115 lines not shown
    return mlp_backward_common("asac_mlp_backward_policy_q", *job, a, nullptr, nullptr, ASAC_MLP_REDUCE_OVERWRITE, nullptr,
                               as_stream(stream));
}

static int backward_policy_sample(const char* where, const asac_mlp_job_t* job, const float* eps, const float* grad_a,
                                  int grad_a_members, const float* log_alpha, const float* off_action,
                                  int64_t off_row_stride, float* grad_params, float* workspace, int reduce_mode,
                                  void* stream) {
    if (!bwd_job_ok(job) || job->E != 1 || job->x1 || job->desc->in1 != 0 || !eps || !grad_a || grad_a_members < 1 ||
        !log_alpha || !grad_params || !workspace)
        return bad_arg(where);
    if (!gauss_head(*job->desc) || job->desc->head_cols[0] > 16) return bad_arg(where);
    MlpArgs a = make_args(*job);
    a.eps = eps;
    a.grad_a = grad_a;
    a.grad_a_members = grad_a_members;
    a.log_alpha = log_alpha;
    a.off_action = off_action;
    a.off_row_stride = off_row_stride;
    return mlp_backward_common(where, *job, a, grad_params, workspace, reduce_mode, nullptr, as_stream(stream));
}

int asac_mlp_backward_policy_sample(const asac_mlp_job_t* job, const float* eps, const float* grad_a, int grad_a_members,
                                    const float* log_alpha, float* grad_params, float* workspace, int reduce_mode,
                                    void* stream) {
    return backward_policy_sample("asac_mlp_backward_policy_sample", job, eps, grad_a, grad_a_members, log_alpha, nullptr, 0,
                                  grad_params, workspace, reduce_mode, stream);
}

int asac_mlp_backward_policy_sample_offline(const asac_mlp_job_t* job, const float* eps, const float* grad_a,
                                            int grad_a_members, const float* log_alpha, const float* off_action,
                                            int64_t off_row_stride, float* grad_params, float* workspace, int reduce_mode,
                                            void* stream) {
    if (!off_action || !job || !job->desc || off_row_stride < job->desc->head_cols[0])
        return bad_arg("asac_mlp_backward_policy_sample_offline: stored actions");
    return backward_policy_sample("asac_mlp_backward_policy_sample_offline", job, eps, grad_a, grad_a_members, log_alpha,
                                  off_action, off_row_stride, grad_params, workspace, reduce_mode, stream);
}

int asac_policy_step_fused_ok(const asac_mlp_desc_t* q_desc, const float* q_params, int64_t q_member_stride,
                              const asac_mlp_desc_t* pi_desc, const float* pi_params, int64_t pi_member_stride, int64_t N) {
    if (!q_desc || !pi_desc || !desc_ok(*q_desc) || !desc_ok(*pi_desc) || N <= 0) return 0;
    if (!stock3(*q_desc, q_params, q_member_stride) || !stock3(*pi_desc, pi_params, pi_member_stride)) return 0;
    if (!scalar_head(*q_desc) || !gauss_head(*pi_desc) || pi_desc->in1 != 0) return 0;
    if (q_desc->in0 != pi_desc->in0 || q_desc->in1 != pi_desc->head_cols[0] || 2 * pi_desc->head_cols[0] > kHeadPad) return 0;
    return mlp_tile_rows(N, 1) == kPsRows ? 1 : 0;
}

static int policy_step_fused(const char* where, const asac_mlp_desc_t* q_desc, const float* q_params, int64_t q_member_stride,
                             const asac_mlp_desc_t* pi_desc, const float* pi_params, int64_t pi_member_stride,
                             const float* x, int64_t x_row_stride, int64_t N, const float* action, const float* eps,
                             const float* log_alpha, const int32_t* subset, const float* off_action, int64_t off_row_stride,
                             float* q_out, float* a_tanh_out, float* logp_out, float* ls_out, float* pi_grad_params,
                             float* workspace, int reduce_mode, void* stream) {
    if (!asac_policy_step_fused_ok(q_desc, q_params, q_member_stride, pi_desc, pi_params, pi_member_stride, N) ||
        !x || !eps || !log_alpha || !pi_grad_params || !workspace || (!action && (!a_tanh_out || !logp_out)))
        return bad_arg(where);
    PolicyStepArgs a{};
    asac_mlp_job_t pi{}, q{};
    pi.desc = pi_desc, pi.params = pi_params, pi.member_stride = pi_member_stride;
    q.desc = q_desc, q.params = q_params, q.member_stride = q_member_stride;
    pi.x0 = q.x0 = x, pi.x0_row_stride = q.x0_row_stride = x_row_stride, pi.N = q.N = N;
    q.x1 = action, q.x1_row_stride = pi_desc->head_cols[0];
    a.q = make_args(q);
    a.pi = make_args(pi);
    if (!offsets32(a.q) || !offsets32(a.pi)) return bad_arg(where);
    a.q.subset = subset;
    a.a_out = a_tanh_out;
    a.logp_out = logp_out;
    a.ls_out = ls_out;
    a.pi.eps = eps;
    a.pi.log_alpha = log_alpha;
    a.pi.partial = workspace;
    a.pi.off_action = off_action;
    a.pi.off_row_stride = off_row_stride;
    a.q_out = q_out;
    static bool attr_done = false, attr_done_offline = false;
    if (int rc = off_action ? set_lds_limit(reinterpret_cast<const void*>(k_policy_step<true>), sizeof(PsLds),
                                            attr_done_offline, where)
                            : set_lds_limit(reinterpret_cast<const void*>(k_policy_step<false>), sizeof(PsLds), attr_done, where))
        return rc;
    const int tiles = (int)((N + kPsRows - 1) / kPsRows);
    hipStream_t s = as_stream(stream);
    if (off_action) ASAC_LAUNCH(k_policy_step<true>, dim3((unsigned)tiles), dim3(kPsThreads), sizeof(PsLds), s, a);
    else ASAC_LAUNCH(k_policy_step<false>, dim3((unsigned)tiles), dim3(kPsThreads), sizeof(PsLds), s, a);
    if (reduce_mode != ASAC_MLP_REDUCE_DEFER)
        reduce_partials(pi_desc, workspace, tiles, 1, pi_member_stride, pi_grad_params, reduce_mode, nullptr, nullptr, 0.f, s);
    return finish_launch(where);
}

int asac_policy_step_fused(const asac_mlp_desc_t* q_desc, const float* q_params, int64_t q_member_stride,
                           const asac_mlp_desc_t* pi_desc, const float* pi_params, int64_t pi_member_stride,
                           const float* x, int64_t x_row_stride, int64_t N, const float* action, const float* eps,
                           const float* log_alpha, const int32_t* subset, float* q_out, float* a_tanh_out,
                           float* logp_out, float* ls_out, float* pi_grad_params, float* workspace, int reduce_mode,
                           void* stream) {
    return policy_step_fused("asac_policy_step_fused", q_desc, q_params, q_member_stride, pi_desc, pi_params,
                             pi_member_stride, x, x_row_stride, N, action, eps, log_alpha, subset, nullptr, 0, q_out,
                             a_tanh_out, logp_out, ls_out, pi_grad_params, workspace, reduce_mode, stream);
}

int asac_policy_step_fused_offline(const asac_mlp_desc_t* q_desc, const float* q_params, int64_t q_member_stride,
                                   const asac_mlp_desc_t* pi_desc, const float* pi_params, int64_t pi_member_stride,
                                   const float* x, int64_t x_row_stride, int64_t N, const float* action, const float* eps,
                                   const float* log_alpha, const int32_t* subset, const float* off_action,
                                   int64_t off_row_stride, float* q_out, float* a_tanh_out, float* logp_out, float* ls_out,
                                   float* pi_grad_params, float* workspace, int reduce_mode, void* stream) {
    if (!off_action || !pi_desc || off_row_stride < pi_desc->head_cols[0])
        return bad_arg("asac_policy_step_fused_offline: stored actions");
    return policy_step_fused("asac_policy_step_fused_offline", q_desc, q_params, q_member_stride, pi_desc, pi_params,
                             pi_member_stride, x, x_row_stride, N, action, eps, log_alpha, subset, off_action,
                             off_row_stride, q_out, a_tanh_out, logp_out, ls_out, pi_grad_params, workspace, reduce_mode,
                             stream);
}

static bool fits32(int64_t v) { return v >= 0 && v < 0x1fffffffLL; }

static StockJobArg stock_job_arg(const asac_mlp_job_t& p) {
    const asac_mlp_desc_t* d = p.desc;
    StockJobArg j{};
    j.P = p.params, j.x0 = p.x0, j.x1 = p.x1, j.out = p.out;
    j.member_stride = (int32_t)p.member_stride, j.N = (int32_t)p.N;
    j.x0_rs = (int32_t)p.x0_row_stride, j.x0_ms = (int32_t)p.x0_member_stride;
    j.x1_rs = (int32_t)p.x1_row_stride, j.x1_ms = (int32_t)p.x1_member_stride;
    j.x0_sb = (int32_t)p.x0_sample_stride, j.x0_T = (int32_t)p.x0_window_T;
    j.in0 = d->in0, j.in1 = d->in1, j.h0 = d->head_cols[0], j.h1 = d->head_cols[1];
    j.hw0 = (int32_t)d->head_w_off[0], j.hw1 = (int32_t)d->head_w_off[1];
    j.hb0 = (int32_t)d->head_b_off[0], j.hb1 = (int32_t)d->head_b_off[1];
    for (int l = 0; l < 3; ++l) {
        j.w_off[l] = (int32_t)d->w_off[l], j.b_off[l] = (int32_t)d->b_off[l];
        j.residual_bits |= (d->residual[l] ? 1 : 0) << l;
    }
    j.head_transform = d->head_transform;
    return j;
}

static asac_mlp_job_t pi_rows(const asac_mlp_job_t& p) {
    asac_mlp_job_t r = p;
    r.x1 = nullptr, r.x1_row_stride = r.x1_member_stride = 0;
    return r;
}

static bool ring_key_ok(const asac_ring_key_t& k, int first_col, int cols) {
    if (!k.src || k.row_bytes <= 0 || k.row_bytes % 4 != 0 || k.row_bytes > (1 << 20) ||
        reinterpret_cast<uintptr_t>(k.src) % 4 != 0)
        return false;
    if (first_col < 0 || cols <= 0 || (int64_t)(first_col + cols) * 4 > k.row_bytes) return false;
    if (k.pad_mode == ASAC_PAD_ROW) return k.pad_row && reinterpret_cast<uintptr_t>(k.pad_row) % 4 == 0;
    return k.pad_mode == ASAC_PAD_KEEP || k.pad_mode == ASAC_PAD_WORD;
}

static bool ring_rows_ok(const asac_pi_q_job_t& j) {
    const asac_ring_rows_t& r = j.ring;
    const asac_squash_job_t& s = j.sample;
    if (!r.ids || !r.index_ring || !is_pow2(r.capacity) || r.prev_n < 0 || r.L <= r.prev_n) return false;
    if (s.T <= 0 || j.pi.N % s.T != 0 || r.j0 < 0 || r.j0 + s.T > r.L) return false;
    if (j.pi.x0_window_T != 0 && j.pi.x0_window_T != s.T) return false;
    if (!ring_key_ok(r.x0, 0, j.pi.desc->in0)) return false;
    if ((s.action || r.x_j0 >= 0) && !ring_key_ok(r.action, 0, 1)) return false;
    if (s.action && !ring_key_ok(r.action, s.action_offset, s.A)) return false;
    return r.x_j0 < r.L;
}

static bool pi_q_job_ok(const asac_pi_q_job_t& j) {
    const asac_mlp_job_t &p = j.pi, &q = j.q;
    if (!p.desc || !q.desc || !desc_ok(*p.desc) || !desc_ok(*q.desc) || p.N <= 0 || q.N != p.N || p.E != 1 || q.E < 1) return false;
// ... 97 lines not shown
                                   ring_attr, "asac_policy_sample_q_forward: hipFuncSetAttribute"))
            return rc;
        if (int rc = set_lds_limit(reinterpret_cast<const void*>(k_pi_sample_q_ring<1>), sizeof(PiQLds), ring_attr1,
                                   "asac_policy_sample_q_forward: hipFuncSetAttribute"))
            return rc;
        const SidecarsDev no_sc{};
        for (int rep = 0; rep < g_launch_repeat; ++rep) {
            const bool last = rep == g_launch_repeat - 1;
            const dim3 grid((unsigned)(m.blocks + blocks + (last ? sc.blocks : 0)));
            if (sc.n <= 1)
                hipLaunchKernelGGL(k_pi_sample_q_ring<1>, grid, dim3(kPiQThreads), sizeof(PiQLds), as_stream(stream), mr,
                                   sidecars_first<1>(last ? sc : no_sc));
            else
                hipLaunchKernelGGL(k_pi_sample_q_ring<ASAC_MAX_SIDECARS>, grid, dim3(kPiQThreads), sizeof(PiQLds),
                                   as_stream(stream), mr, last ? sc : no_sc);
        }
        return finish_launch("asac_policy_sample_q_forward");
    }
    static bool attr_done = false;
    static bool attr_done1 = false;
    if (int rc = set_lds_limit(reinterpret_cast<const void*>(k_pi_sample_q<ASAC_MAX_SIDECARS>), sizeof(PiQLds), attr_done,
                               "asac_policy_sample_q_forward: hipFuncSetAttribute"))
        return rc;
    if (int rc = set_lds_limit(reinterpret_cast<const void*>(k_pi_sample_q<1>), sizeof(PiQLds), attr_done1,
                               "asac_policy_sample_q_forward: hipFuncSetAttribute"))
        return rc;
    const SidecarsDev none{};
    for (int rep = 0; rep < g_launch_repeat; ++rep) {
        const bool last = rep == g_launch_repeat - 1;
        const dim3 grid((unsigned)(m.blocks + blocks + (last ? sc.blocks : 0)));
        if (sc.n <= 1)
            hipLaunchKernelGGL(k_pi_sample_q<1>, grid, dim3(kPiQThreads), sizeof(PiQLds), as_stream(stream), m,
                               sidecars_first<1>(last ? sc : none));
        else
            hipLaunchKernelGGL(k_pi_sample_q<ASAC_MAX_SIDECARS>, grid, dim3(kPiQThreads), sizeof(PiQLds), as_stream(stream), m,
                               last ? sc : none);
    }
    return finish_launch("asac_policy_sample_q_forward");
}

int asac_mlp_backward_qloss_return_ok(const asac_mlp_job_t* job, const asac_vtrace_args_t* ret) {
    if (!job || !job->desc || !desc_ok(*job->desc) || !ret || job->E <= 0 || job->N <= 0 || ret->B != job->N || ret->n <= 0 ||
        !ret->q || !ret->y_out || ret->E_sample <= 0 || ret->E_sample > ASAC_MAX_ENSEMBLE || ret->td_error_out)
        return 0;
    if (wide_input(*job->desc) || !stock3(*job->desc, job->params, job->member_stride)) return 0;
    const int tm = mlp_tile_rows(job->N, job->E);
    const size_t lds = (tm == 16 ? sizeof(MlpBwdLds<16>) : sizeof(MlpBwdLds<32>)) +
                       (size_t)(2 * ((ret->n + 1) | 1) + 2) * tm * sizeof(float) +
                       (tm == 16 && ASAC_BWD_WAVES ? 16 * kP * sizeof(float) : 0);
    const int threads = tm == 16 ? 64 * ASAC_BWD_WAVES : 32 * 16;
    return tm * ret->n <= threads && lds <= 128 * 1024;
}

int asac_mlp_backward_qloss_return(const asac_mlp_job_t* job, const float* target_q, const asac_vtrace_args_t* ret,
                                   const float* weights, float clip_eps, float* loss_out, float* grad_x0, float* grad_params,
                                   float* workspace, int reduce_mode, void* stream) {
    if (!bwd_job_ok(job) || !target_q || !ret || !grad_params || !workspace || clip_eps <= 0.f)
        return bad_arg("asac_mlp_backward_qloss_return");
    if (!scalar_head(*job->desc)) return bad_arg("asac_mlp_backward_qloss_return: not a scalar-head network");
    if (reduce_mode != ASAC_MLP_REDUCE_DEFER && !loss_out) return bad_arg("asac_mlp_backward_qloss_return: loss_out");
    if (!asac_mlp_backward_qloss_return_ok(job, ret) || (ret->use_n_step_is && (!ret->mu_prob || !ret->pi_prob || ret->A <= 0)))
        return bad_arg("asac_mlp_backward_qloss_return: return arguments");
    MlpArgs a = make_args(*job);
    if (!offsets32(a)) return bad_arg("asac_mlp_backward_qloss_return: offsets");
    a.tq = target_q;
    a.y = ret->y_out;
    a.w = weights;
    a.clip_eps = clip_eps;
    a.gx0 = grad_x0;
    RetIn<true> rv{*ret, vtrace_scan_lanes(ret->B, ret->n)};
    return mlp_backward_common("asac_mlp_backward_qloss_return", *job, a, grad_params, workspace, reduce_mode, loss_out,
                               as_stream(stream), &rv);
}

int asac_mlp_backward_qloss(const asac_mlp_job_t* job, const float* target_q, const float* y, const float* weights,
                            float clip_eps, float* loss_out, float* grad_x0, float* grad_params, float* workspace,
                            int reduce_mode, void* stream) {
    if (!bwd_job_ok(job) || !target_q || !y || !grad_params || !workspace || clip_eps <= 0.f)
        return bad_arg("asac_mlp_backward_qloss");
    if (!scalar_head(*job->desc)) return bad_arg("asac_mlp_backward_qloss: not a scalar-head network");
    if (reduce_mode != ASAC_MLP_REDUCE_DEFER && !loss_out) return bad_arg("asac_mlp_backward_qloss: loss_out");
    MlpArgs a = make_args(*job);
    a.tq = target_q;
    a.y = y;
    a.w = weights;
    a.clip_eps = clip_eps;
    a.gx0 = grad_x0;
    return mlp_backward_common("asac_mlp_backward_qloss", *job, a, grad_params, workspace, reduce_mode, loss_out,
                               as_stream(stream));
}

}
```

advanced-soft-actor-critic_amd/native.py:

```python
import ctypes as C
from pathlib import Path

import torch

PKG_DIR = Path(__file__).resolve().parent
import os as _os

LIB_PATH = Path(_os.environ.get('ASAC_HIP_LIB', PKG_DIR / 'lib' / 'libasac_hip.so'))
ABI_VERSION = 91

MAX_GATHER_KEYS = 16
PAD_KEEP, PAD_WORD, PAD_BYTE, PAD_ROW, PAD_EMIT_MASK = 0, 1, 2, 3, 4
CVT_NONE, CVT_U8_TO_F32_UNIT, CVT_BOOL_TO_F32 = 0, 1, 2


class AsacNativeError(RuntimeError):
    pass


class GatherKey(C.Structure):
    _fields_ = [('src', C.c_void_p), ('dst', C.c_void_p), ('pad_row', C.c_void_p),
                ('row_bytes', C.c_int32), ('pad_mode', C.c_int32), ('pad_word', C.c_uint32),
                ('convert', C.c_int32), ('dst_row_pitch', C.c_int32), ('derive', C.c_int32)]

# ... 248 lines not shown
    'asac_sumtree_descend': (C.c_int, [C.c_void_p, C.c_int, C.c_int, C.c_void_p, C.c_void_p, C.c_void_p, C.c_void_p,
                                       C.c_void_p, C.c_void_p]),
    'asac_gather_rows': (C.c_int, [C.POINTER(GatherKey), C.c_int, C.c_void_p, C.c_int, C.c_int, C.c_void_p]),
    'asac_rows_move': (C.c_int, [C.POINTER(RowMove), C.c_int, C.c_void_p, C.c_void_p, C.c_void_p, C.c_int,
                                 C.c_void_p]),
    'asac_batch_put': (C.c_int, [C.POINTER(BatchPutKey), C.c_int, C.c_int, C.c_int, C.c_int, C.c_void_p, C.c_void_p,
                                 C.c_int, C.c_int, C.c_void_p, C.c_void_p, C.c_int, C.c_int, C.c_void_p, C.c_int,
                                 C.c_void_p, C.c_int32, C.c_void_p]),
    'asac_batch_pop_gather': (C.c_int, [C.POINTER(BatchGatherKey), C.c_int, C.c_void_p, C.c_void_p, C.c_int, C.c_int,
                                        C.c_int, C.c_int, C.c_void_p]),
    'asac_window_aux': (C.c_int, [C.c_void_p, C.c_int64, C.c_void_p, C.c_int64, C.c_void_p, C.c_int64, C.c_int64,
                                  C.c_int, C.c_int, C.c_int, C.c_void_p, C.c_void_p, C.c_void_p, C.c_int64, C.c_void_p]),
    'asac_scatter_rows_if_id_match': (C.c_int, [C.c_void_p, C.c_int, C.c_int, C.c_void_p, C.c_int, C.c_int,
                                                C.c_int, C.c_void_p, C.c_void_p, C.c_int, C.c_void_p,
                                                C.c_int64, C.c_int64, C.c_void_p, C.c_void_p]),
    'asac_squash_sample_fwd': (C.c_int, [C.c_void_p, C.c_void_p, C.c_int64, C.c_void_p, C.c_int64, C.c_int,
                                         C.c_void_p, C.c_void_p, C.c_void_p,
                                         C.c_void_p, C.c_int, C.c_int64, C.c_int64, C.c_int,
                                         C.c_void_p, C.c_int64, C.c_int64, C.c_int, C.c_void_p]),
    'asac_squash_sample_bwd': (C.c_int, [C.c_void_p, C.c_void_p, C.c_int64, C.c_void_p, C.c_void_p, C.c_int,
                                         C.c_int64, C.c_void_p, C.c_void_p, C.c_int64, C.c_int, C.c_void_p,
                                         C.c_void_p, C.c_int64, C.c_void_p]),
    'asac_squash_multi': (C.c_int, [C.POINTER(SquashJob), C.c_int, C.POINTER(Sidecar), C.c_int, C.c_void_p]),
    'asac_squash_prob': (C.c_int, [C.c_void_p, C.c_void_p, C.c_int64, C.c_void_p, C.c_int, C.c_int64, C.c_int64,
                                   C.c_int, C.c_int64, C.c_int, C.c_void_p, C.c_int64, C.c_int64, C.c_int,
                                   C.c_void_p]),
    'asac_vtrace_return_min': (C.c_int, [C.POINTER(VtraceArgs), C.c_void_p]),
    'asac_vtrace_return_min_sc': (C.c_int, [C.POINTER(VtraceArgs), C.POINTER(Sidecar), C.c_int, C.POINTER(Sidecar),
                                            C.c_void_p]),
    'asac_td_update': (C.c_int, [C.POINTER(VtraceArgs), C.c_void_p, C.c_int, C.c_void_p, C.c_void_p, C.c_float, C.c_float,
                                 C.c_float, C.c_void_p, C.c_void_p, C.POINTER(Sidecar), C.c_int, C.POINTER(Sidecar),
                                 C.c_void_p]),
    'asac_sumtree_update_sc': (C.c_int, [C.c_void_p, C.c_int, C.c_int, C.c_void_p, C.c_void_p, C.c_void_p, C.c_float,
                                         C.c_float, C.c_float, C.c_int, C.c_void_p, C.c_void_p, C.POINTER(Sidecar), C.c_int,
                                         C.c_void_p]),
    'asac_vtrace_return_direct': (C.c_int, [C.POINTER(VtraceArgs), C.c_void_p, C.c_void_p, C.c_void_p,
                                            C.c_void_p, C.c_void_p]),
    'asac_q_loss_fwd_bwd': (C.c_int, [C.c_void_p, C.c_void_p, C.c_void_p, C.c_void_p, C.c_int, C.c_int,
                                      C.c_float, C.c_void_p, C.c_void_p, C.c_void_p]),
    'asac_mlp_forward': (C.c_int, [C.POINTER(MlpJob), C.c_void_p]),
    'asac_mlp_forward_multi': (C.c_int, [C.POINTER(MlpJob), C.c_int, C.POINTER(Sidecar), C.c_int, C.c_void_p]),
    'asac_mlp_forward_multi_sampled_ok': (C.c_int, [C.POINTER(MlpJob), C.c_int, C.POINTER(SampleEpilogue)]),
    'asac_mlp_forward_multi_sampled': (C.c_int, [C.POINTER(MlpJob), C.c_int, C.POINTER(SampleEpilogue), C.POINTER(Sidecar),
                                                 C.c_int, C.c_void_p]),
    'asac_mlp_backward_workspace': (C.c_int64, [C.c_int64, C.c_int, C.c_int64]),
    'asac_mlp_backward_tiles': (C.c_int64, [C.c_int64, C.c_int]),
    'asac_mlp_backward': (C.c_int, [C.POINTER(MlpJob), C.c_void_p, C.c_void_p, C.c_void_p, C.c_void_p, C.c_void_p, C.c_int,
                                    C.c_void_p]),
    'asac_mlp_backward_qloss': (C.c_int, [C.POINTER(MlpJob), C.c_void_p, C.c_void_p, C.c_void_p, C.c_float, C.c_void_p,
                                          C.c_void_p, C.c_void_p, C.c_void_p, C.c_int, C.c_void_p]),
    'asac_mlp_backward_qloss_return_ok': (C.c_int, [C.POINTER(MlpJob), C.POINTER(VtraceArgs)]),
    'asac_mlp_backward_qloss_return': (C.c_int, [C.POINTER(MlpJob), C.c_void_p, C.POINTER(VtraceArgs), C.c_void_p, C.c_float,
                                                 C.c_void_p, C.c_void_p, C.c_void_p, C.c_void_p, C.c_int, C.c_void_p]),
    'asac_mlp_backward_policy_q': (C.c_int, [C.POINTER(MlpJob), C.c_void_p, C.c_void_p, C.c_int, C.c_void_p, C.c_void_p]),
    'asac_mlp_backward_policy_sample': (C.c_int, [C.POINTER(MlpJob), C.c_void_p, C.c_void_p, C.c_int, C.c_void_p,
                                                  C.c_void_p, C.c_void_p, C.c_int, C.c_void_p]),
    'asac_mlp_backward_policy_sample_offline': (C.c_int, [C.POINTER(MlpJob), C.c_void_p, C.c_void_p, C.c_int, C.c_void_p,
                                                          C.c_void_p, C.c_int64, C.c_void_p, C.c_void_p, C.c_int,
                                                          C.c_void_p]),
    'asac_struct_size': (C.c_int64, [C.c_char_p]),
    'asac_policy_sample_q_forward_ok': (C.c_int, [C.POINTER(PiQJob)]),
    'asac_policy_sample_q_forward_jobs_ok': (C.c_int, [C.POINTER(PiQJob), C.POINTER(MlpJob), C.c_int]),
    'asac_policy_sample_q_forward': (C.c_int, [C.POINTER(PiQJob), C.POINTER(MlpJob), C.c_int, C.POINTER(Sidecar), C.c_int,
                                               C.c_void_p]),
    'asac_policy_step_fused_ok': (C.c_int, [C.POINTER(MlpDesc), C.c_void_p, C.c_int64, C.POINTER(MlpDesc), C.c_void_p,
                                            C.c_int64, C.c_int64]),
    'asac_policy_step_fused': (C.c_int, [C.POINTER(MlpDesc), C.c_void_p, C.c_int64, C.POINTER(MlpDesc), C.c_void_p,
                                         C.c_int64, C.c_void_p, C.c_int64, C.c_int64, C.c_void_p, C.c_void_p,
                                         C.c_void_p, C.c_void_p, C.c_void_p, C.c_void_p, C.c_void_p, C.c_void_p,
                                         C.c_void_p, C.c_void_p, C.c_int, C.c_void_p]),
    'asac_policy_step_fused_offline': (C.c_int, [C.POINTER(MlpDesc), C.c_void_p, C.c_int64, C.POINTER(MlpDesc), C.c_void_p,
                                                 C.c_int64, C.c_void_p, C.c_int64, C.c_int64, C.c_void_p, C.c_void_p,
                                                 C.c_void_p, C.c_void_p, C.c_void_p, C.c_int64, C.c_void_p, C.c_void_p,
                                                 C.c_void_p, C.c_void_p, C.c_void_p, C.c_void_p, C.c_int, C.c_void_p]),
    'asac_policy_offline_term': (C.c_int, [C.c_void_p, C.c_void_p, C.c_int64, C.c_void_p, C.c_void_p, C.c_int64, C.c_int,
                                           C.c_int, C.c_void_p, C.c_void_p, C.c_void_p]),
    'asac_mlp_param_extent': (C.c_int64, [C.POINTER(MlpDesc)]),
    'asac_adam_step_partials': (C.c_int, [C.c_void_p, C.c_void_p, C.c_void_p, C.c_void_p, C.c_float, C.c_float,
                                          C.c_float, C.c_float, C.c_void_p, C.c_void_p, C.c_int64, C.c_int,
                                          C.c_int64, C.c_int64, C.c_int, C.c_void_p, C.c_int64, C.c_void_p]),
    'asac_gauss_head_fwd': (C.c_int, [C.c_void_p, C.c_int64, C.c_int, C.c_void_p, C.c_void_p, C.c_void_p]),
    'asac_gauss_head_bwd': (C.c_int, [C.c_void_p, C.c_void_p, C.c_void_p, C.c_int64, C.c_int, C.c_void_p,
                                      C.c_void_p]),
    'asac_attention_supported': (C.c_int, [C.c_int, C.c_int, C.c_int]),
    'asac_attention_forward': (C.c_int, [C.c_void_p, C.c_void_p, C.c_void_p, C.c_void_p, C.c_int64, C.c_int64, C.c_int64,
                                         C.c_int, C.c_int, C.c_int, C.c_int, C.c_void_p, C.c_void_p, C.c_void_p,
                                         C.c_void_p]),
    'asac_attention_backward': (C.c_int, [C.c_void_p, C.c_void_p, C.c_void_p, C.c_void_p, C.c_void_p, C.c_void_p, C.c_int,
                                          C.c_int, C.c_int, C.c_int, C.c_void_p, C.c_void_p, C.c_void_p, C.c_void_p]),
    'asac_attention_proj_workspace': (C.c_int64, [C.c_int, C.c_int, C.c_int, C.c_int]),
    'asac_attention_proj_forward': (C.c_int, [C.c_void_p, C.c_int64, C.c_int64, C.c_void_p, C.c_int64, C.c_int64,
                                              C.c_void_p * 8, C.c_void_p, C.c_int64, C.c_int64, C.c_int64, C.c_int,
                                              C.c_int, C.c_int, C.c_int, C.c_void_p, C.c_void_p, C.c_void_p, C.c_void_p,
                                              C.c_void_p, C.c_int64, C.c_int64, C.c_void_p]),
    'asac_attention_proj_backward': (C.c_int, [C.c_void_p, C.c_int64, C.c_int64, C.c_void_p, C.c_int64, C.c_int64,
                                               C.c_void_p * 8, C.c_void_p, C.c_void_p, C.c_void_p, C.c_void_p, C.c_int64,
                                               C.c_int64, C.c_void_p, C.c_void_p, C.c_int64, C.c_int64,
                                               C.c_int, C.c_int, C.c_int, C.c_int, C.c_void_p, C.c_void_p, C.c_void_p,
                                               C.c_int, C.c_void_p, C.c_void_p]),
    'asac_linear_tanh_workspace': (C.c_int64, [C.c_int64, C.c_int, C.c_int]),
    'asac_linear_tanh_forward': (C.c_int, [C.c_void_p, C.c_int64, C.c_void_p, C.c_void_p, C.c_int64, C.c_int, C.c_int,
                                           C.c_void_p, C.c_void_p]),
    'asac_linear_tanh_backward': (C.c_int, [C.c_void_p, C.c_int64, C.c_void_p, C.c_void_p, C.c_void_p, C.c_int64, C.c_int,
                                            C.c_int, C.c_void_p, C.c_void_p, C.c_int, C.c_void_p, C.c_void_p]),
    'asac_linear_tanh_forward2': (C.c_int, [C.c_void_p, C.c_int64, C.c_int, C.c_void_p, C.c_int64, C.c_int, C.c_void_p,
                                            C.c_void_p, C.c_int64, C.c_int, C.c_void_p, C.c_void_p]),
# ... 878 lines not shown
    extra_jobs = list(extra_jobs)
    assert len(extra_jobs) <= MLP_MAX_JOBS
    arr = (MlpJob * len(extra_jobs))(*extra_jobs) if extra_jobs else None
    sc, n_sc = _sidecar_array(sidecars)
    _check(load().asac_policy_sample_q_forward(C.byref(job), arr, len(extra_jobs), sc, n_sc, _stream()),
           'asac_policy_sample_q_forward')


def mlp_backward_workspace(member_stride, E, N) -> int:
    return int(load().asac_mlp_backward_workspace(member_stride, E, N))


def mlp_backward_tiles(N, E) -> int:
    return int(load().asac_mlp_backward_tiles(N, E))


MLP_REDUCE_OVERWRITE, MLP_REDUCE_ACCUMULATE, MLP_REDUCE_DEFER = 0, 1, 2


def mlp_param_extent(desc) -> int:
    return int(load().asac_mlp_param_extent(C.byref(desc)))


@_profiled
def mlp_backward_qloss(job: MlpJob, target_q, y, weights, clip_eps, loss_out, grad_params, workspace, reduce_mode,
                       grad_x0=None):
    global _last_work
    _last_work = _pass_flops(job, backward=True)
    E, N = job.E, job.N
    assert target_q.is_contiguous() and target_q.numel() == E * N and y.is_contiguous() and y.numel() == N
    assert grad_x0 is None or (grad_x0.is_contiguous() and grad_x0.numel() == E * N * job.desc.contents.in0)
    _check(load().asac_mlp_backward_qloss(C.byref(job), _p(target_q), _p(y), _p(weights), float(clip_eps), _p(loss_out),
                                          _p(grad_x0), _p(grad_params), _p(workspace), int(reduce_mode), _stream()),
           'asac_mlp_backward_qloss')


def mlp_backward_qloss_return_ok(job: MlpJob, ret: VtraceArgs) -> bool:
    return bool(load().asac_mlp_backward_qloss_return_ok(C.byref(job), C.byref(ret)))


@_profiled
def mlp_backward_qloss_return(job: MlpJob, target_q, ret: VtraceArgs, weights, clip_eps, loss_out, grad_params, workspace,
                              reduce_mode, grad_x0=None):
    global _last_work
    _last_work = _pass_flops(job, backward=True)
    E, N = job.E, job.N
    assert target_q.is_contiguous() and target_q.numel() == E * N
    assert grad_x0 is None or (grad_x0.is_contiguous() and grad_x0.numel() == E * N * job.desc.contents.in0)
    _check(load().asac_mlp_backward_qloss_return(C.byref(job), _p(target_q), C.byref(ret), _p(weights), float(clip_eps),
                                                 _p(loss_out), _p(grad_x0), _p(grad_params), _p(workspace), int(reduce_mode),
                                                 _stream()), 'asac_mlp_backward_qloss_return')


@_profiled
def mlp_backward_policy_q(job: MlpJob, q_table, subset, E_sample, grad_x1):
    global _last_work
    _last_work = _pass_flops(job, backward=True, param_grads=False)
    assert q_table.is_contiguous() and q_table.numel() == job.E * job.N and grad_x1.is_contiguous()
    _check(load().asac_mlp_backward_policy_q(C.byref(job), _p(q_table), _p(subset), E_sample, _p(grad_x1), _stream()),
           'asac_mlp_backward_policy_q')


def _offline_view(offline, N, A):
    assert offline.dtype == torch.float32 and tuple(offline.shape) == (N, A), 'offline: [N, A] float32 stored actions'
    assert offline.stride(1) == 1, 'offline: the action dimension must be contiguous'
    assert N == 1 or offline.stride(0) >= A, 'offline: overlapping rows'
    return _p(offline), (offline.stride(0) if N > 1 else max(offline.stride(0), A))


def _mlp_backward_policy_sample(job: MlpJob, eps, grad_a, log_alpha, grad_params, workspace, reduce_mode):
    global _last_work
    _last_work = _pass_flops(job, backward=True)
    N, A = job.N, job.desc.contents.head_cols[0]
    assert eps.is_contiguous() and eps.numel() == N * A and grad_a.is_contiguous() and grad_a.numel() % (N * A) == 0
    _check(load().asac_mlp_backward_policy_sample(C.byref(job), _p(eps), _p(grad_a), grad_a.numel() // (N * A),
                                                  _p(log_alpha), _p(grad_params), _p(workspace), int(reduce_mode),
                                                  _stream()), 'asac_mlp_backward_policy_sample')


_mlp_backward_policy_sample = _profiled(_mlp_backward_policy_sample, 'asac_mlp_backward_policy_sample')


@_profiled
def mlp_backward_policy_sample_offline(job: MlpJob, eps, grad_a, log_alpha, offline, grad_params, workspace, reduce_mode):
    global _last_work
    _last_work = _pass_flops(job, backward=True)
    N, A = job.N, job.desc.contents.head_cols[0]
    assert eps.is_contiguous() and eps.numel() == N * A and grad_a.is_contiguous() and grad_a.numel() % (N * A) == 0
    po, rso = _offline_view(offline, N, A)
    _check(load().asac_mlp_backward_policy_sample_offline(C.byref(job), _p(eps), _p(grad_a), grad_a.numel() // (N * A),
                                                          _p(log_alpha), po, rso, _p(grad_params), _p(workspace),
                                                          int(reduce_mode), _stream()),
           'asac_mlp_backward_policy_sample_offline')


def mlp_backward_policy_sample(job: MlpJob, eps, grad_a, log_alpha, grad_params, workspace, reduce_mode, offline=None):
    if offline is None:
        return _mlp_backward_policy_sample(job, eps, grad_a, log_alpha, grad_params, workspace, reduce_mode)
    return mlp_backward_policy_sample_offline(job, eps, grad_a, log_alpha, offline, grad_params, workspace, reduce_mode)


def policy_step_fused_ok(q_desc, q_params, q_member_stride, pi_desc, pi_params, pi_member_stride, N) -> bool:
    return bool(load().asac_policy_step_fused_ok(C.byref(q_desc), _p(q_params), q_member_stride, C.byref(pi_desc),
                                                 _p(pi_params), pi_member_stride, N))


# ... 2 lines not shown
                      ls_out=None, offline=None):
    if offline is not None:
        _offline_view(offline, N, pi_desc.head_cols[0])
        return policy_step_fused_offline(q_desc, q_params, q_member_stride, pi_desc, pi_params, pi_member_stride, x, N,
                                         action, eps, log_alpha, q_out, pi_grad_params, workspace, reduce_mode, subset,
                                         a_out, logp_out, ls_out, offline)
    return _policy_step_fused_plain(q_desc, q_params, q_member_stride, pi_desc, pi_params, pi_member_stride, x, N, action,
                                    eps, log_alpha, q_out, pi_grad_params, workspace, reduce_mode, subset, a_out, logp_out,
                                    ls_out)


@_profiled
def policy_step_fused_offline(q_desc, q_params, q_member_stride, pi_desc, pi_params, pi_member_stride, x, N, action, eps,
                              log_alpha, q_out, pi_grad_params, workspace, reduce_mode, subset, a_out, logp_out, ls_out,
                              offline):
    return _policy_step_fused(q_desc, q_params, q_member_stride, pi_desc, pi_params, pi_member_stride, x, N, action, eps,
                              log_alpha, q_out, pi_grad_params, workspace, reduce_mode, subset, a_out, logp_out, ls_out,
                              offline)


def _policy_step_fused(q_desc, q_params, q_member_stride, pi_desc, pi_params, pi_member_stride, x, N, action, eps,
                       log_alpha, q_out, pi_grad_params, workspace, reduce_mode, subset=None, a_out=None, logp_out=None,
                       ls_out=None, offline=None):
    global _last_work
    _last_work = (mlp_flops(q_desc, 2, N, backward=True, param_grads=False)
                  + mlp_flops(pi_desc, 1, N, backward=True, param_grads=True))
    p0, rs0, _ = _rows_view(x)
    A = pi_desc.head_cols[0]
    assert eps.is_contiguous() and eps.numel() == N * A
    if action is not None:
        assert action.is_contiguous() and action.numel() == N * A
    else:
        assert a_out.is_contiguous() and a_out.numel() == N * A and logp_out.is_contiguous() and logp_out.numel() == N
        assert ls_out is None or (ls_out.is_contiguous() and ls_out.numel() == 2 * N * A)
    assert q_out is None or (q_out.is_contiguous() and q_out.numel() % N == 0 and q_out.numel() >= 2 * N)
    assert subset is None or (subset.dtype == torch.int32 and subset.numel() == 2)
    if offline is not None:
        po, rso = _offline_view(offline, N, A)
        _check(load().asac_policy_step_fused_offline(C.byref(q_desc), _p(q_params), q_member_stride, C.byref(pi_desc),
                                                     _p(pi_params), pi_member_stride, p0, rs0, N, _p(action), _p(eps),
                                                     _p(log_alpha), _p(subset), po, rso, _p(q_out), _p(a_out),
                                                     _p(logp_out), _p(ls_out), _p(pi_grad_params), _p(workspace),
                                                     int(reduce_mode), _stream()),
               'asac_policy_step_fused_offline')
        return
    _check(load().asac_policy_step_fused(C.byref(q_desc), _p(q_params), q_member_stride, C.byref(pi_desc), _p(pi_params),
                                         pi_member_stride, p0, rs0, N, _p(action), _p(eps), _p(log_alpha), _p(subset),
                                         _p(q_out), _p(a_out), _p(logp_out), _p(ls_out), _p(pi_grad_params), _p(workspace),
                                         int(reduce_mode), _stream()),
           'asac_policy_step_fused')


_policy_step_fused_plain = _profiled(_policy_step_fused, 'asac_policy_step_fused')


@_profiled
def adam_step_partials(param, grad, exp_avg, exp_avg_sq, lr, beta1, beta2, eps, steps_done, workspace, tiles, E,
                       member_stride, used, accumulate, loss_out=None, loss_rows=0):
    assert param.numel() >= E * member_stride and steps_done.dtype == torch.int64
    _check(load().asac_adam_step_partials(_p(param), _p(grad), _p(exp_avg), _p(exp_avg_sq), lr, beta1, beta2, eps,
                                          _p(steps_done), _p(workspace), tiles, E, member_stride, used,
                                          int(bool(accumulate)), _p(loss_out), loss_rows, _stream()),
           'asac_adam_step_partials')


@_profiled
def mlp_backward(job: MlpJob, grad_out, grad_x0, grad_x1, grad_params, workspace, reduce_mode=MLP_REDUCE_ACCUMULATE):
    global _last_work
    _last_work = _pass_flops(job, backward=True, param_grads=grad_params is not None)
    _check(load().asac_mlp_backward(C.byref(job), _p(grad_out), _p(grad_x0), _p(grad_x1), _p(grad_params), _p(workspace),
                                    int(reduce_mode), _stream()), 'asac_mlp_backward')


def attention_supported(Lq: int, Lk: int, D: int) -> bool:
    return bool(load().asac_attention_supported(int(Lq), int(Lk), int(D)))


@_profiled
def attention_forward(q, k, v, mask, out, weights, keep):
    _dense_f32(q, k, v, out, weights, keep)
    B, Lq, D = q.shape
    sb = si = sj = 0
    if mask is not None:
        assert mask.element_size() == 1 and mask.dim() == 3
        sb, si, sj = (0 if mask.shape[d] == 1 else mask.stride(d) for d in range(3))
    _check(load().asac_attention_forward(_p(q), _p(k), _p(v), _p(mask), sb, si, sj, B, Lq, k.shape[1], D, _p(out),
                                         _p(weights), _p(keep), _stream()), 'asac_attention_forward')


@_profiled
def attention_backward(q, k, v, weights, grad_out, grad_weights, grad_q, grad_k, grad_v):
    _dense_f32(q, k, v, weights, grad_out, grad_weights, grad_q, grad_k, grad_v)
    B, Lq, D = q.shape
    _check(load().asac_attention_backward(_p(q), _p(k), _p(v), _p(weights), _p(grad_out), _p(grad_weights), B, Lq,
                                          k.shape[1], D, _p(grad_q), _p(grad_k), _p(grad_v), _stream()),
           'asac_attention_backward')


def _proj_ptrs(params):
    assert len(params) in (6, 8)
    arr = (C.c_void_p * 8)()
    for i, t in enumerate(params):
        assert t.is_cuda and t.is_contiguous() and t.dtype == torch.float32
        arr[i] = t.data_ptr()
    return arr

# ... 1846 lines not shown
```

include/asac_hip.h:

```cpp
#ifndef ASAC_HIP_H
#define ASAC_HIP_H

#include <stdint.h>

#ifdef __cplusplus
extern "C" {
#endif

#define ASAC_ABI_VERSION 91
#define ASAC_MAX_GATHER_KEYS 16
#define ASAC_MAX_ENSEMBLE 16
#define ASAC_MAX_ACTION 64
#define ASAC_MLP_MAX_BLOCKS 4

int asac_version(void);
int64_t asac_struct_size(const char* name);
const char* asac_last_error(void);

int asac_set_launch_repeat(int repeat);


int asac_sumtree_sample(const float* tree, int capacity, int batch, const double* u,
                        const int64_t* slot_ids, double* beta_state, double beta_increment,
                        int32_t* leaf_out, float* p_out, int64_t* ids_out, float* is_weights_out,
// ... 269 lines not shown
                                   const asac_sidecar_t* sidecars_host, int n_sidecars, void* stream);

typedef struct {
    const void* src;
    const void* pad_row;
    int32_t row_bytes;
    int32_t pad_mode;
    uint32_t pad_word;
    int32_t reserved_;
} asac_ring_key_t;
typedef struct {
    const int64_t* ids;
    const int32_t* index_ring;
    int32_t capacity, prev_n, L;
    int32_t j0;
    int32_t x_j0;
    int32_t x_action_offset;
    asac_ring_key_t x0, action;
} asac_ring_rows_t;
typedef struct {
    asac_mlp_job_t pi;
    asac_squash_job_t sample;
    const float* eps2;
    int32_t t2;
    int32_t reserved_;
    float* a2_out;
    float* logp2_out;
    asac_mlp_job_t q;
    asac_ring_rows_t ring;
} asac_pi_q_job_t;
int asac_policy_sample_q_forward_ok(const asac_pi_q_job_t* job);
int asac_policy_sample_q_forward_jobs_ok(const asac_pi_q_job_t* job, const asac_mlp_job_t* extra_jobs, int n_extra);
int asac_policy_sample_q_forward(const asac_pi_q_job_t* job, const asac_mlp_job_t* extra_jobs, int n_extra,
                                 const asac_sidecar_t* sidecars_host, int n_sidecars, void* stream);

#define ASAC_MLP_REDUCE_OVERWRITE 0
#define ASAC_MLP_REDUCE_ACCUMULATE 1
#define ASAC_MLP_REDUCE_DEFER 2
int64_t asac_mlp_backward_workspace(int64_t member_stride, int E, int64_t N);
int64_t asac_mlp_backward_tiles(int64_t N, int E);

int asac_mlp_backward(const asac_mlp_job_t* job, const float* grad_out, float* grad_x0, float* grad_x1, float* grad_params,
                      float* workspace, int reduce_mode, void* stream);

int asac_mlp_backward_qloss(const asac_mlp_job_t* job, const float* target_q, const float* y, const float* weights,
                            float clip_eps, float* loss_out, float* grad_x0, float* grad_params, float* workspace,
                            int reduce_mode, void* stream);

int asac_mlp_backward_qloss_return_ok(const asac_mlp_job_t* job, const asac_vtrace_args_t* ret);
int asac_mlp_backward_qloss_return(const asac_mlp_job_t* job, const float* target_q, const asac_vtrace_args_t* ret,
                                   const float* weights, float clip_eps, float* loss_out, float* grad_x0, float* grad_params,
                                   float* workspace, int reduce_mode, void* stream);

int asac_mlp_backward_policy_q(const asac_mlp_job_t* job, const float* q_table, const int32_t* subset, int E_sample,
                               float* grad_x1, void* stream);

int asac_policy_step_fused_ok(const asac_mlp_desc_t* q_desc, const float* q_params, int64_t q_member_stride,
                              const asac_mlp_desc_t* pi_desc, const float* pi_params, int64_t pi_member_stride, int64_t N);
int asac_policy_step_fused(const asac_mlp_desc_t* q_desc, const float* q_params, int64_t q_member_stride,
                           const asac_mlp_desc_t* pi_desc, const float* pi_params, int64_t pi_member_stride,
                           const float* x, int64_t x_row_stride, int64_t N, const float* action, const float* eps,
                           const float* log_alpha, const int32_t* subset, float* q_out, float* a_tanh_out,
                           float* logp_out, float* ls_out, float* pi_grad_params, float* workspace, int reduce_mode,
                           void* stream);
int asac_policy_step_fused_offline(const asac_mlp_desc_t* q_desc, const float* q_params, int64_t q_member_stride,
                                   const asac_mlp_desc_t* pi_desc, const float* pi_params, int64_t pi_member_stride,
                                   const float* x, int64_t x_row_stride, int64_t N, const float* action, const float* eps,
                                   const float* log_alpha, const int32_t* subset, const float* off_action,
                                   int64_t off_row_stride, float* q_out, float* a_tanh_out, float* logp_out, float* ls_out,
                                   float* pi_grad_params, float* workspace, int reduce_mode, void* stream);

int asac_mlp_backward_policy_sample(const asac_mlp_job_t* job, const float* eps, const float* grad_a, int grad_a_members,
                                    const float* log_alpha, float* grad_params, float* workspace, int reduce_mode,
                                    void* stream);
int asac_mlp_backward_policy_sample_offline(const asac_mlp_job_t* job, const float* eps, const float* grad_a,
                                            int grad_a_members, const float* log_alpha, const float* off_action,
                                            int64_t off_row_stride, float* grad_params, float* workspace, int reduce_mode,
                                            void* stream);

int64_t asac_mlp_param_extent(const asac_mlp_desc_t* desc_host);

int asac_gauss_head_fwd(const float* raw, int64_t rows, int A, float* loc, float* scale, void* stream);
int asac_gauss_head_bwd(const float* raw, const float* grad_loc, const float* grad_scale,
                        int64_t rows, int A, float* grad_raw, void* stream);

#define ASAC_GRU_MAX_LAYERS 2
#define ASAC_GRU_MAX_DIM 16
typedef struct {
    int32_t input, hidden, hidden_pow2, layers;
} asac_gru_desc_t;

int64_t asac_gru_param_count(const asac_gru_desc_t* desc_host);
int64_t asac_gru_backward_workspace(const asac_gru_desc_t* desc_host, int B);

int asac_gru_forward(const asac_gru_desc_t* desc_host, const float* const* w_ih, const float* const* w_hh,
                     const float* const* b_ih, const float* const* b_hh, const float* x,
                     int64_t x_stride_b, int64_t x_stride_t, const float* h0, int64_t h0_stride_b,
                     const uint8_t* padding_mask, int64_t mask_stride_b, int B, int L, float* hn_out,
                     float* out_top, float* gates_out, void* stream);

int asac_gru_forward_twin(const asac_gru_desc_t* desc_host, const float* const* w_ih, const float* const* w_hh,
                          const float* const* b_ih, const float* const* b_hh, const float* const* twin_w_ih,
                          const float* const* twin_w_hh, const float* const* twin_b_ih,
                          const float* const* twin_b_hh, const float* x, int64_t x_stride_b, int64_t x_stride_t,
                          const float* h0, int64_t h0_stride_b, const uint8_t* padding_mask,
                          int64_t mask_stride_b, int B, int L, float* hn_out, float* out_top, float* gates_out,
                          float* twin_hn_out, float* twin_out_top, void* stream);

int asac_gru_backward(const asac_gru_desc_t* desc_host, const float* const* w_ih, const float* const* w_hh,
                      const float* const* b_ih, const float* const* b_hh, const float* x,
                      int64_t x_stride_b, int64_t x_stride_t, const float* h0, int64_t h0_stride_b,
                      const uint8_t* padding_mask, int64_t mask_stride_b, int B, int L, const float* hn,
                      const float* gates, const float* grad_hn, const float* grad_top, float* grad_x,
                      float* grad_h0, float* grad_params, float* const* grad_param_tensors, int accumulate,
                      float* workspace, void* stream);

typedef struct {
    float* param_base;
    const float* grad_base;
    float* exp_avg_base;
    float* exp_avg_sq_base;
    float lr, beta1, beta2, eps;
    const int64_t* steps_done;
// ... 616 lines not shown
```

Baseline: 12620 train_steps/s.

## Ride policy forward on spare workgroups of critic backward, reuse it in policy step

```diff
diff --git a/advanced-soft-actor-critic_amd/algorithm/fused_mlp.py b/advanced-soft-actor-critic_amd/algorithm/fused_mlp.py
--- a/advanced-soft-actor-critic_amd/algorithm/fused_mlp.py
+++ b/advanced-soft-actor-critic_amd/algorithm/fused_mlp.py
@@ -318,6 +318,7 @@
         self._anchor = torch.zeros(1, device=device, requires_grad=True)
         self.accumulate = True
         self._workspace = None
+        self._forward_saves = {}
         self._start, self._deferred_rows = start, None
         self.device = device
 
@@ -373,6 +374,26 @@
         self._deferred_rows = N if defer else None
         return g0
 
+    def forward_save_buffer(self, N: int):
+        buf = self._forward_saves.get(N)
+        if buf is None:
+            buf = self._forward_saves[N] = torch.zeros(native.policy_forward_save_floats(N), dtype=torch.float32, device=self.device)
+        return buf
+
+    def backward_qloss_return_rider_ok(self, N: int, ret, policy: 'StockMLP', x_pi, save) -> bool:
+        return (policy.E == 1 and x_pi.dim() == 2 and
+                native.mlp_backward_qloss_return_rider_ok(self._pass(None, None, N=N), ret, policy._pass(x_pi, None), save))
+
+    def backward_qloss_return_rider(self, x0, x1, target_q, ret, weights, clip_eps, loss_out, policy: 'StockMLP', x_pi, save,
+                                    defer=False, state_grads=False):
+        N = x0.shape[-2]
+        g0 = torch.empty((self.E, N, self.in0), dtype=torch.float32, device=self.device) if state_grads else None
+        native.mlp_backward_qloss_return_rider(self._pass(x0, x1), target_q, ret, weights, clip_eps, loss_out,
+                                               self.grad_params, self._workspace_for(N), self._reduce_mode(defer),
+                                               policy._pass(x_pi, None), save, grad_x0=g0)
+        self._deferred_rows = N if defer else None
+        return g0
+
     def backward_policy_q(self, x0, x1, q_table, subset, E_sample):
         N = x0.shape[-2]
         g1 = torch.empty((self.E, N, self.in1), dtype=torch.float32, device=self.device)
@@ -399,6 +420,15 @@
                                  self.member_stride, x0, N, action, eps, log_alpha, q_out, self.grad_params,
                                  self._workspace_for(N), self._reduce_mode(defer), subset=subset, a_out=a_out,
                                  logp_out=logp_out, ls_out=ls_out, offline=offline)
+        self._deferred_rows = N if defer else None
+
+    def policy_step_fused_loaded(self, critics: 'StockMLP', x0, action, eps, log_alpha, saved, q_out=None, defer=False,
+                                 subset=None, offline=None):
+        N = x0.shape[-2]
+        assert subset is not None or critics.E == 2
+        native.policy_step_fused_loaded(critics.desc, critics.params, critics.member_stride, self.desc, self.params,
+                                        self.member_stride, x0, N, action, eps, log_alpha, saved, q_out, self.grad_params,
+                                        self._workspace_for(N), self._reduce_mode(defer), subset=subset, offline=offline)
         self._deferred_rows = N if defer else None
 
     def adam_partials(self, opt, loss_out=None):
diff --git a/advanced-soft-actor-critic_amd/algorithm/sac_base.py b/advanced-soft-actor-critic_amd/algorithm/sac_base.py
--- a/advanced-soft-actor-critic_amd/algorithm/sac_base.py
+++ b/advanced-soft-actor-critic_amd/algorithm/sac_base.py
@@ -277,6 +277,7 @@
         self._fused_td_chain = bool(hip_config.get('fused_td_chain', True))
         self._fused_td_update = bool(hip_config.get('fused_td_update', True))
         self._fused_q_return = bool(hip_config.get('fused_q_return', True))
+        self._policy_forward_rider = bool(hip_config.get('policy_forward_rider', True))
         self._fused_q_state_grads = bool(hip_config.get('fused_q_state_grads', True))
         self._gru_backward_at = bool(hip_config.get('gru_backward_at', True))
         self._adjacent_cat = bool(hip_config.get('adjacent_cat', True))
@@ -544,6 +545,8 @@
         self._discrete_grads = {}
         self._hybrid_bufs = {}
         self._ls_y = None
+        self._pi_saved = None
+        self._rider_plan_cache = None
         self._cq_buf, self._tq_buf, self._cq_td_buf = (torch.zeros(E, B, 1, **f32) for _ in range(3))
         self._pi_q, self._pi_stats_src = torch.zeros(E, B, 1, **f32), None
         self._pi_a, self._pi_logp, self._pi_sampled = torch.zeros(B, A1, **f32), torch.zeros(B, **f32), False
@@ -1411,12 +1414,35 @@
                                   launch=False)
         return c_y, ret
 
-    def _stock_q_backward(self, x0, a0, ret, c_y, priority_is, fold, fused_return, state_grads=False):
+    def _rider_plan(self, x_pi, ret):
+        key = (x_pi.data_ptr(), x_pi.stride(0), x_pi.shape[0], ret.args.n)
+        cached = self._rider_plan_cache
+        if cached is not None and cached[0] == key:
+            return cached[1]
+        B, fq, fpi = x_pi.shape[0], self._fq, self._fpi
+        save = None
+        if self._fused_policy_step and self.ensemble_q_sample == 2 and fpi.policy_step_fused_ok(fq, B):
+            save = fpi.forward_save_buffer(B)
+            if not (fq.backward_qloss_return_rider_ok(B, ret.args, fpi, x_pi, save) and
+                    native.policy_step_fused_loaded_ok(fq.desc, fq.params, fq.member_stride, fpi.desc, fpi.params,
+                                                       fpi.member_stride, B, save)):
+                save = None
+        self._rider_plan_cache = (key, save)
+        return save
+
+    def _stock_q_backward(self, x0, a0, ret, c_y, priority_is, fold, fused_return, state_grads=False, rider_rows=None):
         w = priority_is.reshape(-1).contiguous() if priority_is is not None else None
         t_q = self._tq_buf.view(self.ensemble_q_num, -1)
+        self._pi_saved = None
         if fused_return and self._fq.backward_qloss_return_ok(x0.shape[-2], ret.args):
-            g0 = self._fq.backward_qloss_return(x0, a0, t_q, ret.args, w, self.clip_epsilon, self._loss_q_e,
-                                                defer=fold, state_grads=state_grads)
+            save = self._rider_plan(rider_rows, ret) if rider_rows is not None else None
+            if save is not None:
+                g0 = self._fq.backward_qloss_return_rider(x0, a0, t_q, ret.args, w, self.clip_epsilon, self._loss_q_e,
+                                                          self._fpi, rider_rows, save, defer=fold, state_grads=state_grads)
+                self._pi_saved = (save, rider_rows.data_ptr(), rider_rows.stride(0), rider_rows.shape[0])
+            else:
+                g0 = self._fq.backward_qloss_return(x0, a0, t_q, ret.args, w, self.clip_epsilon, self._loss_q_e,
+                                                    defer=fold, state_grads=state_grads)
         else:
             self._launch_return(ret)
             g0 = self._fq.backward_qloss(x0, a0, t_q, c_y.reshape(-1), w, self.clip_epsilon, self._loss_q_e,
@@ -1470,7 +1496,9 @@
             c_y, ret = self._stock_q_targets(job_tq, job_pi, ls, window, policy_sample)
         opt = self.optimizer_q_list[0]
         fold = self._dist is None and opt.start == self._fq._start and self._params.span('rep')[0] == self._params.span('rep')[1]
-        self._stock_q_backward(x0, a0, ret, c_y, priority_is, fold, fused_return=fused is not None and self._fused_q_return)
+        rider_rows = x0 if (self._policy_forward_rider and fused is not None and policy_sample and x0.dim() == 2) else None
+        self._stock_q_backward(x0, a0, ret, c_y, priority_is, fold, fused_return=fused is not None and self._fused_q_return,
+                               rider_rows=rider_rows)
         if not fold:
             self._finish_rep_q(None, None)
 
@@ -1687,6 +1715,7 @@
         B = x.shape[0]
         fusable = (self._fused_policy_step and self.ensemble_q_sample == 2 and self._fpi.policy_step_fused_ok(self._fq, B))
         sample_out = None
+        saved, self._pi_saved, given = self._pi_saved, None, False
         if ls is None and not self._pi_sampled and fusable:
             f32 = dict(dtype=torch.float32, device=self.device)
             self.noise.normal_(self._eps_pi)
@@ -1697,7 +1726,7 @@
                 ls = self._fpi._launch_forward(x, None)[0]
             loc, scale = ls[..., :A], ls[..., A:]
             if self._pi_sampled:
-                a_tanh, logp, self._pi_sampled = self._pi_a, self._pi_logp, False
+                a_tanh, logp, self._pi_sampled, given = self._pi_a, self._pi_logp, False, True
             else:
                 self.noise.normal_(self._eps_pi)
                 a_tanh = torch.empty((B, A), dtype=torch.float32, device=self.device)
@@ -1709,7 +1738,12 @@
             logp, scale, sample_out[2] if sample_out is not None else ls, self._eps_pi, offline)
         opt = self.optimizer_policy
         fold = self._dist is None and (opt.start, opt.stop) == (self._fpi._start, self._fpi._start + self._fpi.member_stride)
-        if fusable and a_tanh.is_contiguous():
+        if (fusable and given and saved is not None and a_tanh.is_contiguous()
+                and saved[1:] == (x.data_ptr(), x.stride(0), B)):
+            self._fpi.policy_step_fused_loaded(self._fq, x, a_tanh, self._eps_pi, self.log_c_alpha, saved[0],
+                                               q_out=self._pi_q, defer=fold, subset=sub if E != 2 else None,
+                                               offline=offline)
+        elif fusable and a_tanh.is_contiguous():
             self._fpi.policy_step_fused(self._fq, x, None if sample_out is not None else a_tanh, self._eps_pi,
                                         self.log_c_alpha, q_out=self._pi_q, defer=fold, subset=sub if E != 2 else None,
                                         sample_out=sample_out, offline=offline)
diff --git a/advanced-soft-actor-critic_amd/csrc/mlp.hip b/advanced-soft-actor-critic_amd/csrc/mlp.hip
--- a/advanced-soft-actor-critic_amd/csrc/mlp.hip
+++ b/advanced-soft-actor-critic_amd/csrc/mlp.hip
@@ -5,6 +5,8 @@
 #include "asac_vtrace.h"
 
 #include <cmath>
+#include <string>
+#include <type_traits>
 
 namespace asac {
 
@@ -890,14 +892,31 @@
     int32_t seg;
 };
 
-template <int TM, bool WIDE, int NB, bool RET = false, int W8 = 0>
-__global__ __launch_bounds__(W8 ? 64 * W8 : TM * 16) void k_mlp_bwd(const MlpArgs a, const RetIn<RET> rv) {
+template <bool RIDER>
+struct RiderIn {};
+template <>
+struct RiderIn<true>;
+__device__ __forceinline__ void policy_forward_rider(const ASAC_KARG RiderIn<true>& rd, unsigned char* smem);
+template <bool RET>
+constexpr size_t rider_karg_offset();
+
+template <int TM, bool WIDE, int NB, bool RET = false, int W8 = 0, bool RIDER = false>
+__global__ __launch_bounds__(W8 ? 64 * W8 : TM * 16) void k_mlp_bwd(const MlpArgs a, const RetIn<RET> rv, const RiderIn<RIDER> rider_by_value) {
     static_assert(W8 == 0 || ((W8 == 8 || W8 == 16) && TM == 16 && NB == 3 && !WIDE), "8 / 16 waves: 16-row tiles of the stock networks");
+    static_assert(!RIDER || (RET && W8 == 16), "the rider's workgroups are k_policy_step's: 16 waves on a 16-row tile");
     constexpr int THREADS = W8 ? 64 * W8 : threads_of<TM>();
     constexpr int RT = TM / 16;
     constexpr bool fixed = NB > 0;
     static_assert(!(fixed && WIDE), "the fixed-shape path has a first layer of <= 64 inputs");
     extern __shared__ __attribute__((aligned(16))) unsigned char smem_raw[];
+    if constexpr (RIDER) {
+        if (blockIdx.z != 0) {
+            policy_forward_rider(*reinterpret_cast<const ASAC_KARG RiderIn<true>*>(
+                                     static_cast<const ASAC_KARG unsigned char*>(kernarg_base()) + rider_karg_offset<RET>()),
+                                 smem_raw);
+            return;
+        }
+    }
     MlpBwdLds<TM>& L = *reinterpret_cast<MlpBwdLds<TM>*>(smem_raw);
     const int e = blockIdx.y;
     const int64_t row0 = (int64_t)blockIdx.x * TM;
@@ -1271,12 +1290,34 @@
 };
 static_assert(sizeof(PsPiLds) <= 2 * sizeof(PsQLds), "the policy phase reuses the critics' LDS");
 
+struct SavedPolicyTile {
+    float x[3][kPsRows * kMaxW];
+    f32x4 zp[3][4 * 64];
+    float head[kPsRows * kHeadPad];
+};
+static_assert(sizeof(SavedPolicyTile) == 25600, "SavedPolicyTile");
+constexpr int kSavedTileFloats = sizeof(SavedPolicyTile) / sizeof(float);
+struct PsParked {
+    float x[3][kPsRows * kP];
+    f32x4 zp[3][4 * 64];
+    float head[kPsRows * kHeadPad];
+};
+struct PsLdsLoaded {
+    PsLds l;
+    PsParked k;
+};
+static_assert(sizeof(PsLds) % 16 == 0 && offsetof(PsParked, zp) % 16 == 0, "the parked fragments are read 16 bytes a lane");
+static_assert(sizeof(PsLdsLoaded) <= 160 * 1024, "one workgroup per CU: the whole LDS");
+
 struct PolicyStepArgs {
     MlpArgs q, pi;
     float* q_out;
     float* a_out;
     float* logp_out;
     float* ls_out;
+};
+struct PolicyStepArgsLoaded : PolicyStepArgs {
+    const float* saved;
 };
 
 __device__ __forceinline__ void ps_fetch_tile(const StageScalars& q, int64_t row0, float (&v)[kPsSlots]) {
@@ -1302,12 +1343,15 @@
     }
 }
 
-template <bool OFFLINE>
-__global__ __launch_bounds__(kPsThreads) void k_policy_step(const PolicyStepArgs a_by_value) {
+template <bool OFFLINE, bool LOADED = false>
+__global__ __launch_bounds__(kPsThreads) void k_policy_step(
+    const std::conditional_t<LOADED, PolicyStepArgsLoaded, PolicyStepArgs> a_by_value) {
     extern __shared__ __attribute__((aligned(16))) unsigned char smem_raw[];
-    const ASAC_KARG PolicyStepArgs& a = *static_cast<const ASAC_KARG PolicyStepArgs*>(kernarg_base());
+    using Args = std::conditional_t<LOADED, PolicyStepArgsLoaded, PolicyStepArgs>;
+    const ASAC_KARG Args& a = *static_cast<const ASAC_KARG Args*>(kernarg_base());
     PsLds& L = *reinterpret_cast<PsLds*>(smem_raw);
     PsPiLds& P = *reinterpret_cast<PsPiLds*>(smem_raw);
+    [[maybe_unused]] PsParked& K = reinterpret_cast<PsLdsLoaded*>(smem_raw)->k;
     const int wave = threadIdx.x >> 6, lane = threadIdx.x & 63;
     const int m = wave >> 2, ct = wave & 3;
     const int col = ct * 16 + (lane & 15);
@@ -1319,13 +1363,23 @@
 
     const int e0 = a.q.subset ? a.q.subset[0] : 0, e1 = a.q.subset ? a.q.subset[1] : 1;
     const StageScalars s0 = stage_scalars<3>(a.q, e0), s1 = stage_scalars<3>(a.q, e1), sp = stage_scalars<3>(a.pi, 0);
-    const bool sample_here = a.q.x1 == nullptr;
+    const bool sample_here = !LOADED && a.q.x1 == nullptr;
     float in_q[kPsSlots] = {}, in_pi[kPsSlots];
     if (!sample_here) ps_fetch_tile(s0, row0, in_q);
     ps_fetch_tile(sp, row0, in_pi);
     StagedNet<kPsThreads> r0, r1, rp;
     net_fetch_fixed<kPsThreads, 3>(s0, r0);
     net_fetch_fixed<kPsThreads, 3>(s1, r1);
+    [[maybe_unused]] float sv_x[3], sv_h;
+    [[maybe_unused]] f32x4 sv_z;
+    if constexpr (LOADED) {
+        static_assert(kPsThreads == 1024, "the parked tile is dealt over sixteen waves");
+        const SavedPolicyTile& sv = *reinterpret_cast<const SavedPolicyTile*>(a.saved + (int64_t)blockIdx.x * kSavedTileFloats);
+#pragma unroll
+        for (int l = 0; l < 3; ++l) sv_x[l] = sv.x[l][threadIdx.x];
+        sv_z = (&sv.zp[0][0])[threadIdx.x < 768 ? threadIdx.x : 767];
+        sv_h = sv.head[threadIdx.x & 255];
+    }
     net_fetch_fixed<kPsThreads, 3>(sp, rp);
     float ev = 0.f, gl = 0.f;
     {
@@ -1397,6 +1451,12 @@
     }
     net_put_fixed<kPsThreads, 3>(r0, L.q[0]);
     net_put_fixed<kPsThreads, 3>(r1, L.q[1]);
+    if constexpr (LOADED) {
+#pragma unroll
+        for (int l = 0; l < 3; ++l) K.x[l][(threadIdx.x >> 6) * kP + (threadIdx.x & 63)] = sv_x[l];
+        (&K.zp[0][0])[threadIdx.x < 768 ? threadIdx.x : 767] = sv_z;
+        K.head[threadIdx.x & 255] = sv_h;
+    }
     __syncthreads();
     if (sample_here) {
         if ((int)threadIdx.x < kPsRows * A) {
@@ -1490,11 +1550,19 @@
 
     net_put_fixed<kPsThreads, 3>(rp, P);
     ps_put_tile(in_pi, P.x[0]);
-    if (threadIdx.x < kPsRows * kHeadPad) P.delta[(threadIdx.x >> 4) * kP + (threadIdx.x & 15)] = 0.f;
+    if (threadIdx.x < kPsRows * kHeadPad)
+        P.delta[(threadIdx.x >> 4) * kP + (threadIdx.x & 15)] = LOADED ? K.head[threadIdx.x] : 0.f;
     loads_landed();
     __syncthreads();
     MLP_STAMP(6);
+    const float* const px[4] = {P.x[0], LOADED ? K.x[0] : P.x[1], LOADED ? K.x[1] : P.x[2], LOADED ? K.x[2] : P.x[3]};
     f32x4 zp[3];
+    if constexpr (LOADED) {
+        if (wave < 4) {
+#pragma unroll
+            for (int l = 0; l < 3; ++l) zp[l] = K.zp[l][threadIdx.x];
+        }
+    } else {
 #pragma unroll
     for (int l = 0; l < 3; ++l) {
         if (wave < 4) {
@@ -1527,6 +1595,7 @@
         for (int r = 0; r < 4; ++r) P.delta[(4 * (lane >> 4) + r) * kP + hc] = raw[r] + P.head_bias[hc];
     }
     __syncthreads();
+    }
     MLP_STAMP(8);
     if ((int)threadIdx.x < kPsRows * A) {
         const int lrow = threadIdx.x / A, d = threadIdx.x - lrow * A;
@@ -1553,8 +1622,8 @@
     __syncthreads();
     MLP_STAMP(9);
     float* part = a.pi.partial + (int64_t)blockIdx.x * a.pi.member_stride;
-    ps_grad_weight(P.delta, 0, P.x[3], A, kMaxW, part + a.pi.d.head_w_off[0]);
-    ps_grad_weight(P.delta, A, P.x[3], A, kMaxW, part + a.pi.d.head_w_off[1], 4);
+    ps_grad_weight(P.delta, 0, px[3], A, kMaxW, part + a.pi.d.head_w_off[0]);
+    ps_grad_weight(P.delta, A, px[3], A, kMaxW, part + a.pi.d.head_w_off[1], 4);
     if (wave == 7) {
         const int c = lane & 15, rq = (lane >> 4) * 4;
         float sb = 0.f;
@@ -1580,7 +1649,7 @@
             for (int r = 0; r < 4; ++r) pdelta[(4 * (lane >> 4) + r) * kP + pc] = gp[r] * zp[l][r];
         }
         __syncthreads();
-        ps_grad_weight(pdelta, 0, P.x[l], kMaxW, Kin, part + a.pi.d.w_off[l]);
+        ps_grad_weight(pdelta, 0, px[l], kMaxW, Kin, part + a.pi.d.w_off[l]);
         grad_bias<kPsRows>(pdelta, 0, kMaxW, part + a.pi.d.b_off[l]);
         if (l > 0 && wave < 4) {
             f32x4 gin = gemm_tile_nt(pdelta, P.w[l], kMaxW, 0, wave);
@@ -1695,6 +1764,70 @@
 #pragma unroll
     for (int l = 0; l < 3; ++l) { ASAC_PIN(q.w_off[l]); ASAC_PIN(q.b_off[l]); }
     return q;
+}
+
+template <>
+struct RiderIn<true> {
+    StockJobArg pi;
+    float* save;
+};
+template <bool RET>
+constexpr size_t rider_karg_offset() {
+    constexpr size_t a1 = alignof(RetIn<RET>), a2 = alignof(RiderIn<true>);
+    return ((((sizeof(MlpArgs) + a1 - 1) / a1 * a1) + sizeof(RetIn<RET>)) + a2 - 1) / a2 * a2;
+}
+__device__ __forceinline__ void policy_forward_rider(const ASAC_KARG RiderIn<true>& rd, unsigned char* smem) {
+    PsPiLds& P = *reinterpret_cast<PsPiLds*>(smem);
+    const int wave = threadIdx.x >> 6, lane = threadIdx.x & 63;
+    const int tile = blockIdx.x + blockIdx.y * gridDim.x;
+    const StageScalars sp = stage_scalars_stock(rd.pi, 0);
+    const int64_t row0 = (int64_t)tile * kPsRows;
+    if (row0 >= sp.N) return;
+    SavedPolicyTile& out = *reinterpret_cast<SavedPolicyTile*>(rd.save + (int64_t)tile * kSavedTileFloats);
+    const int K0p = sp.in0;
+    const int residual_bits = rd.pi.residual_bits;
+    float in_pi[kPsSlots];
+    ps_fetch_tile(sp, row0, in_pi);
+    StagedNet<kPsThreads> rp;
+    net_fetch_fixed<kPsThreads, 3>(sp, rp);
+    net_put_fixed<kPsThreads, 3>(rp, P);
+    ps_put_tile(in_pi, P.x[0]);
+    __syncthreads();
+#pragma unroll
+    for (int l = 0; l < 3; ++l) {
+        if (wave < 4) {
+            const float* xin = P.x[l];
+            float* xout = P.x[l + 1];
+            const f32x4 acc = l > 0 ? gemm_tile(xin, P.w[l], kMaxW, 0, wave) : gemm_tile(xin, P.w[l], round4(K0p), 0, wave);
+            const int pc = wave * 16 + (lane & 15);
+            const float bias = P.bias[l][pc];
+            const bool res = ((residual_bits >> l) & 1) != 0;
+            f32x2_g ya, yb, da, db;
+            gelu_parts2((f32x2_g){acc[0] + bias, acc[1] + bias}, ya, da);
+            gelu_parts2((f32x2_g){acc[2] + bias, acc[3] + bias}, yb, db);
+            const float yv[4] = {ya.x, ya.y, yb.x, yb.y};
+            out.zp[l][threadIdx.x] = f32x4{da.x, da.y, db.x, db.y};
+#pragma unroll
+            for (int r = 0; r < 4; ++r) {
+                const int row = 4 * (lane >> 4) + r;
+                float y = yv[r];
+                if (res) y += xin[row * kP + pc];
+                xout[row * kP + pc] = y;
+            }
+        }
+        __syncthreads();
+    }
+    if (wave == 0) {
+        const f32x4 raw = gemm_tile(P.x[3], P.head, kMaxW, 0, 0);
+        const int hc = lane & 15;
+#pragma unroll
+        for (int r = 0; r < 4; ++r) out.head[(4 * (lane >> 4) + r) * kHeadPad + hc] = raw[r] + P.head_bias[hc];
+    }
+#pragma unroll
+    for (int l = 0; l < 3; ++l) {
+        const int r = threadIdx.x >> 6, c = threadIdx.x & 63;
+        out.x[l][r * kMaxW + c] = P.x[l + 1][r * kP + c];
+    }
 }
 
 template <bool WINDOW, bool RING = false, bool SINGLE = false>
@@ -2322,8 +2455,8 @@
 #endif
 template <int TM>
 static int launch_backward(const char* where, const asac_mlp_desc_t* desc, MlpArgs& a, int E, int tiles, hipStream_t s,
-                           const RetIn<true>* ret = nullptr) {
-    static bool attr_done = false, attr_wide = false, attr_stock = false, attr_ret = false;
+                           const RetIn<true>* ret = nullptr, const RiderIn<true>* rider = nullptr) {
+    static bool attr_done = false, attr_wide = false, attr_stock = false, attr_ret = false, attr_rider = false;
     const bool wide = wide_input(*desc);
     const bool stock = !wide && stock3(*desc, a.params, a.member_stride) && offsets32(a);
     constexpr int w8 = TM == 16 ? ASAC_BWD_WAVES : 0;
@@ -2331,7 +2464,7 @@
     auto launch = [&](auto kernel, bool& attr, size_t lds_limit, int threads, size_t lds,
                       const auto& ret_in) -> int {
         if (int rc = set_lds_limit(reinterpret_cast<const void*>(kernel), lds_limit, attr, where)) return rc;
-        ASAC_LAUNCH(kernel, dim3(tiles, E), dim3(threads), lds, s, a, ret_in);
+        ASAC_LAUNCH(kernel, dim3(tiles, E), dim3(threads), lds, s, a, ret_in, RiderIn<false>{});
         return 0;
     };
     const size_t lds = sizeof(MlpBwdLds<TM>);
@@ -2339,6 +2472,17 @@
     if (ret) {
         const size_t lds_ret = lds + (size_t)(2 * ((ret->v.n + 1) | 1) + 2) * TM * sizeof(float) + spare;
         if (!stock || TM * ret->v.n > stock_threads || lds_ret > 128 * 1024) return bad_arg(where);
+        if (rider) {
+            if constexpr (w8 == 16 && kPsThreads == 64 * w8) {
+                auto kernel = k_mlp_bwd<TM, false, 3, true, w8, true>;
+                if (int rc = set_lds_limit(reinterpret_cast<const void*>(kernel), 128 * 1024, attr_rider, where)) return rc;
+                const size_t lds_both = lds_ret > sizeof(PsPiLds) ? lds_ret : sizeof(PsPiLds);
+                ASAC_LAUNCH(kernel, dim3(tiles, E, 2), dim3(stock_threads), lds_both, s, a, *ret, *rider);
+                return 0;
+            } else {
+                return bad_arg(where);
+            }
+        }
         return launch(k_mlp_bwd<TM, false, 3, true, w8>, attr_ret, 128 * 1024, stock_threads, lds_ret, *ret);
     }
     if (wide) return launch(k_mlp_bwd<TM, true, 0>, attr_wide, lds, threads_of<TM>(), lds, RetIn<false>{});
@@ -2361,16 +2505,31 @@
 }
 
 static int mlp_backward_common(const char* where, const asac_mlp_job_t& j, MlpArgs& a, float* grad_params, float* workspace,
-                               int reduce_mode, float* loss_out, hipStream_t s, const RetIn<true>* ret = nullptr) {
+                               int reduce_mode, float* loss_out, hipStream_t s, const RetIn<true>* ret = nullptr,
+                               const RiderIn<true>* rider = nullptr) {
     const int tiles = (int)asac_mlp_backward_tiles(j.N, j.E);
     a.partial = grad_params ? workspace : nullptr;
     a.loss_partial = workspace ? workspace + (int64_t)tiles * j.E * j.member_stride : nullptr;
-    if (int rc = mlp_tile_rows(j.N, j.E) == 16 ? launch_backward<16>(where, j.desc, a, j.E, tiles, s, ret)
-                                               : launch_backward<32>(where, j.desc, a, j.E, tiles, s, ret))
+    if (int rc = mlp_tile_rows(j.N, j.E) == 16 ? launch_backward<16>(where, j.desc, a, j.E, tiles, s, ret, rider)
+                                               : launch_backward<32>(where, j.desc, a, j.E, tiles, s, ret, rider))
         return rc;
     if (grad_params && reduce_mode != ASAC_MLP_REDUCE_DEFER)
         reduce_partials(j.desc, workspace, tiles, j.E, j.member_stride, grad_params, reduce_mode,
                         loss_out ? a.loss_partial : nullptr, loss_out, 1.f / (float)j.N, s);
+    return finish_launch(where);
+}
+
+template <bool OFFLINE, bool LOADED, typename ARGS>
+static int launch_policy_step(const char* where, const ARGS& args, const asac_mlp_desc_t* pi_desc, int64_t pi_member_stride,
+                              int64_t N, float* pi_grad_params, float* workspace, int reduce_mode, hipStream_t s) {
+    static bool attr_done = false;
+    constexpr size_t lds = LOADED ? sizeof(PsLdsLoaded) : sizeof(PsLds);
+    auto kernel = k_policy_step<OFFLINE, LOADED>;
+    if (int rc = set_lds_limit(reinterpret_cast<const void*>(kernel), lds, attr_done, where)) return rc;
+    const int tiles = (int)((N + kPsRows - 1) / kPsRows);
+    ASAC_LAUNCH(kernel, dim3((unsigned)tiles), dim3(kPsThreads), lds, s, args);
+    if (reduce_mode != ASAC_MLP_REDUCE_DEFER)
+        reduce_partials(pi_desc, workspace, tiles, 1, pi_member_stride, pi_grad_params, reduce_mode, nullptr, nullptr, 0.f, s);
     return finish_launch(where);
 }
 
@@ -2592,11 +2751,11 @@
                              const float* x, int64_t x_row_stride, int64_t N, const float* action, const float* eps,
                              const float* log_alpha, const int32_t* subset, const float* off_action, int64_t off_row_stride,
                              float* q_out, float* a_tanh_out, float* logp_out, float* ls_out, float* pi_grad_params,
-                             float* workspace, int reduce_mode, void* stream) {
+                             float* workspace, int reduce_mode, void* stream, const float* saved = nullptr) {
     if (!asac_policy_step_fused_ok(q_desc, q_params, q_member_stride, pi_desc, pi_params, pi_member_stride, N) ||
-        !x || !eps || !log_alpha || !pi_grad_params || !workspace || (!action && (!a_tanh_out || !logp_out)))
+        !x || !eps || !log_alpha || !pi_grad_params || !workspace || (!action && (saved || !a_tanh_out || !logp_out)))
         return bad_arg(where);
-    PolicyStepArgs a{};
+    PolicyStepArgsLoaded a{};
     asac_mlp_job_t pi{}, q{};
     pi.desc = pi_desc, pi.params = pi_params, pi.member_stride = pi_member_stride;
     q.desc = q_desc, q.params = q_params, q.member_stride = q_member_stride;
@@ -2615,18 +2774,14 @@
     a.pi.off_action = off_action;
     a.pi.off_row_stride = off_row_stride;
     a.q_out = q_out;
-    static bool attr_done = false, attr_done_offline = false;
-    if (int rc = off_action ? set_lds_limit(reinterpret_cast<const void*>(k_policy_step<true>), sizeof(PsLds),
-                                            attr_done_offline, where)
-                            : set_lds_limit(reinterpret_cast<const void*>(k_policy_step<false>), sizeof(PsLds), attr_done, where))
-        return rc;
-    const int tiles = (int)((N + kPsRows - 1) / kPsRows);
+    a.saved = saved;
+    const PolicyStepArgs& plain = a;
     hipStream_t s = as_stream(stream);
-    if (off_action) ASAC_LAUNCH(k_policy_step<true>, dim3((unsigned)tiles), dim3(kPsThreads), sizeof(PsLds), s, a);
-    else ASAC_LAUNCH(k_policy_step<false>, dim3((unsigned)tiles), dim3(kPsThreads), sizeof(PsLds), s, a);
-    if (reduce_mode != ASAC_MLP_REDUCE_DEFER)
-        reduce_partials(pi_desc, workspace, tiles, 1, pi_member_stride, pi_grad_params, reduce_mode, nullptr, nullptr, 0.f, s);
-    return finish_launch(where);
+    if (saved)
+        return off_action ? launch_policy_step<true, true>(where, a, pi_desc, pi_member_stride, N, pi_grad_params, workspace, reduce_mode, s)
+                          : launch_policy_step<false, true>(where, a, pi_desc, pi_member_stride, N, pi_grad_params, workspace, reduce_mode, s);
+    return off_action ? launch_policy_step<true, false>(where, plain, pi_desc, pi_member_stride, N, pi_grad_params, workspace, reduce_mode, s)
+                      : launch_policy_step<false, false>(where, plain, pi_desc, pi_member_stride, N, pi_grad_params, workspace, reduce_mode, s);
 }
 
 int asac_policy_step_fused(const asac_mlp_desc_t* q_desc, const float* q_params, int64_t q_member_stride,
@@ -2652,6 +2807,40 @@
                              pi_member_stride, x, x_row_stride, N, action, eps, log_alpha, subset, off_action,
                              off_row_stride, q_out, a_tanh_out, logp_out, ls_out, pi_grad_params, workspace, reduce_mode,
                              stream);
+}
+
+int asac_policy_step_fused_loaded_ok(const asac_mlp_desc_t* q_desc, const float* q_params, int64_t q_member_stride,
+                                     const asac_mlp_desc_t* pi_desc, const float* pi_params, int64_t pi_member_stride, int64_t N,
+                                     const float* saved) {
+    if (!saved || (reinterpret_cast<uintptr_t>(saved) & 15) || kPsThreads != 1024) return 0;
+    return asac_policy_step_fused_ok(q_desc, q_params, q_member_stride, pi_desc, pi_params, pi_member_stride, N);
+}
+
+int asac_policy_step_fused_loaded(const asac_mlp_desc_t* q_desc, const float* q_params, int64_t q_member_stride,
+                                  const asac_mlp_desc_t* pi_desc, const float* pi_params, int64_t pi_member_stride,
+                                  const float* x, int64_t x_row_stride, int64_t N, const float* action, const float* eps,
+                                  const float* log_alpha, const int32_t* subset, const float* saved, float* q_out,
+                                  float* pi_grad_params, float* workspace, int reduce_mode, void* stream) {
+    if (!action || !asac_policy_step_fused_loaded_ok(q_desc, q_params, q_member_stride, pi_desc, pi_params, pi_member_stride, N, saved))
+        return bad_arg("asac_policy_step_fused_loaded");
+    return policy_step_fused("asac_policy_step_fused_loaded", q_desc, q_params, q_member_stride, pi_desc, pi_params,
+                             pi_member_stride, x, x_row_stride, N, action, eps, log_alpha, subset, nullptr, 0, q_out, nullptr,
+                             nullptr, nullptr, pi_grad_params, workspace, reduce_mode, stream, saved);
+}
+
+int asac_policy_step_fused_loaded_offline(const asac_mlp_desc_t* q_desc, const float* q_params, int64_t q_member_stride,
+                                          const asac_mlp_desc_t* pi_desc, const float* pi_params, int64_t pi_member_stride,
+                                          const float* x, int64_t x_row_stride, int64_t N, const float* action,
+                                          const float* eps, const float* log_alpha, const int32_t* subset,
+                                          const float* off_action, int64_t off_row_stride, const float* saved, float* q_out,
+                                          float* pi_grad_params, float* workspace, int reduce_mode, void* stream) {
+    if (!off_action || !pi_desc || off_row_stride < pi_desc->head_cols[0])
+        return bad_arg("asac_policy_step_fused_loaded_offline: stored actions");
+    if (!action || !asac_policy_step_fused_loaded_ok(q_desc, q_params, q_member_stride, pi_desc, pi_params, pi_member_stride, N, saved))
+        return bad_arg("asac_policy_step_fused_loaded_offline");
+    return policy_step_fused("asac_policy_step_fused_loaded_offline", q_desc, q_params, q_member_stride, pi_desc, pi_params,
+                             pi_member_stride, x, x_row_stride, N, action, eps, log_alpha, subset, off_action, off_row_stride,
+                             q_out, nullptr, nullptr, nullptr, pi_grad_params, workspace, reduce_mode, stream, saved);
 }
 
 static bool fits32(int64_t v) { return v >= 0 && v < 0x1fffffffLL; }
@@ -2855,25 +3044,61 @@
     return tm * ret->n <= threads && lds <= 128 * 1024;
 }
 
-int asac_mlp_backward_qloss_return(const asac_mlp_job_t* job, const float* target_q, const asac_vtrace_args_t* ret,
-                                   const float* weights, float clip_eps, float* loss_out, float* grad_x0, float* grad_params,
-                                   float* workspace, int reduce_mode, void* stream) {
-    if (!bwd_job_ok(job) || !target_q || !ret || !grad_params || !workspace || clip_eps <= 0.f)
-        return bad_arg("asac_mlp_backward_qloss_return");
-    if (!scalar_head(*job->desc)) return bad_arg("asac_mlp_backward_qloss_return: not a scalar-head network");
-    if (reduce_mode != ASAC_MLP_REDUCE_DEFER && !loss_out) return bad_arg("asac_mlp_backward_qloss_return: loss_out");
+int64_t asac_policy_forward_save_floats(int64_t N) { return N > 0 ? (N + kPsRows - 1) / kPsRows * kSavedTileFloats : 0; }
+
+int asac_mlp_backward_qloss_return_rider_ok(const asac_mlp_job_t* job, const asac_vtrace_args_t* ret,
+                                            const asac_mlp_job_t* pi_job, const float* save) {
+    if (!pi_job || !save || !asac_mlp_backward_qloss_return_ok(job, ret)) return 0;
+    if (mlp_tile_rows(job->N, job->E) != kPsRows || 64 * ASAC_BWD_WAVES != kPsThreads) return 0;
+    const asac_mlp_job_t& p = *pi_job;
+    if (!p.desc || !desc_ok(*p.desc) || p.N <= 0 || p.E != 1 || !p.x0 || p.x0_window_T != 0) return 0;
+    if (!stock3(*p.desc, p.params, p.member_stride) || !gauss_head(*p.desc) || p.desc->in1 != 0 ||
+        2 * p.desc->head_cols[0] > kHeadPad)
+        return 0;
+    if (!job_fits32(p) || !fits32(p.member_stride) || (reinterpret_cast<uintptr_t>(save) & 15)) return 0;
+    return (p.N + kPsRows - 1) / kPsRows <= asac_mlp_backward_tiles(job->N, job->E) * job->E ? 1 : 0;
+}
+
+static int backward_qloss_return(const char* where, const asac_mlp_job_t* job, const float* target_q,
+                                 const asac_vtrace_args_t* ret, const float* weights, float clip_eps, float* loss_out,
+                                 float* grad_x0, float* grad_params, float* workspace, int reduce_mode,
+                                 const asac_mlp_job_t* pi_job, float* save, void* stream) {
+    auto refuse = [&](const char* why) { return bad_arg((std::string(where) + why).c_str()); };
+    if (!bwd_job_ok(job) || !target_q || !ret || !grad_params || !workspace || clip_eps <= 0.f) return refuse("");
+    if (!scalar_head(*job->desc)) return refuse(": not a scalar-head network");
+    if (reduce_mode != ASAC_MLP_REDUCE_DEFER && !loss_out) return refuse(": loss_out");
     if (!asac_mlp_backward_qloss_return_ok(job, ret) || (ret->use_n_step_is && (!ret->mu_prob || !ret->pi_prob || ret->A <= 0)))
-        return bad_arg("asac_mlp_backward_qloss_return: return arguments");
+        return refuse(": return arguments");
     MlpArgs a = make_args(*job);
-    if (!offsets32(a)) return bad_arg("asac_mlp_backward_qloss_return: offsets");
+    if (!offsets32(a)) return refuse(": offsets");
     a.tq = target_q;
     a.y = ret->y_out;
     a.w = weights;
     a.clip_eps = clip_eps;
     a.gx0 = grad_x0;
     RetIn<true> rv{*ret, vtrace_scan_lanes(ret->B, ret->n)};
-    return mlp_backward_common("asac_mlp_backward_qloss_return", *job, a, grad_params, workspace, reduce_mode, loss_out,
-                               as_stream(stream), &rv);
+    if (pi_job) {
+        RiderIn<true> rd{stock_job_arg(pi_rows(*pi_job)), save};
+        return mlp_backward_common(where, *job, a, grad_params, workspace, reduce_mode, loss_out, as_stream(stream), &rv, &rd);
+    }
+    return mlp_backward_common(where, *job, a, grad_params, workspace, reduce_mode, loss_out, as_stream(stream), &rv);
+}
+
+int asac_mlp_backward_qloss_return(const asac_mlp_job_t* job, const float* target_q, const asac_vtrace_args_t* ret,
+                                   const float* weights, float clip_eps, float* loss_out, float* grad_x0, float* grad_params,
+                                   float* workspace, int reduce_mode, void* stream) {
+    return backward_qloss_return("asac_mlp_backward_qloss_return", job, target_q, ret, weights, clip_eps, loss_out, grad_x0,
+                                 grad_params, workspace, reduce_mode, nullptr, nullptr, stream);
+}
+
+int asac_mlp_backward_qloss_return_rider(const asac_mlp_job_t* job, const float* target_q, const asac_vtrace_args_t* ret,
+                                         const float* weights, float clip_eps, float* loss_out, float* grad_x0,
+                                         float* grad_params, float* workspace, int reduce_mode, const asac_mlp_job_t* pi_job,
+                                         float* save, void* stream) {
+    if (!asac_mlp_backward_qloss_return_rider_ok(job, ret, pi_job, save))
+        return bad_arg("asac_mlp_backward_qloss_return_rider: the policy job");
+    return backward_qloss_return("asac_mlp_backward_qloss_return_rider", job, target_q, ret, weights, clip_eps, loss_out,
+                                 grad_x0, grad_params, workspace, reduce_mode, pi_job, save, stream);
 }
 
 int asac_mlp_backward_qloss(const asac_mlp_job_t* job, const float* target_q, const float* y, const float* weights,
diff --git a/advanced-soft-actor-critic_amd/native.py b/advanced-soft-actor-critic_amd/native.py
--- a/advanced-soft-actor-critic_amd/native.py
+++ b/advanced-soft-actor-critic_amd/native.py
@@ -324,6 +324,23 @@
     'asac_mlp_backward_qloss_return_ok': (C.c_int, [C.POINTER(MlpJob), C.POINTER(VtraceArgs)]),
     'asac_mlp_backward_qloss_return': (C.c_int, [C.POINTER(MlpJob), C.c_void_p, C.POINTER(VtraceArgs), C.c_void_p, C.c_float,
                                                  C.c_void_p, C.c_void_p, C.c_void_p, C.c_void_p, C.c_int, C.c_void_p]),
+    'asac_policy_forward_save_floats': (C.c_int64, [C.c_int64]),
+    'asac_mlp_backward_qloss_return_rider_ok': (C.c_int, [C.POINTER(MlpJob), C.POINTER(VtraceArgs), C.POINTER(MlpJob),
+                                                          C.c_void_p]),
+    'asac_mlp_backward_qloss_return_rider': (C.c_int, [C.POINTER(MlpJob), C.c_void_p, C.POINTER(VtraceArgs), C.c_void_p,
+                                                       C.c_float, C.c_void_p, C.c_void_p, C.c_void_p, C.c_void_p, C.c_int,
+                                                       C.POINTER(MlpJob), C.c_void_p, C.c_void_p]),
+    'asac_policy_step_fused_loaded_ok': (C.c_int, [C.POINTER(MlpDesc), C.c_void_p, C.c_int64, C.POINTER(MlpDesc), C.c_void_p,
+                                                   C.c_int64, C.c_int64, C.c_void_p]),
+    'asac_policy_step_fused_loaded': (C.c_int, [C.POINTER(MlpDesc), C.c_void_p, C.c_int64, C.POINTER(MlpDesc), C.c_void_p,
+                                                C.c_int64, C.c_void_p, C.c_int64, C.c_int64, C.c_void_p, C.c_void_p,
+                                                C.c_void_p, C.c_void_p, C.c_void_p, C.c_void_p, C.c_void_p, C.c_void_p,
+                                                C.c_int, C.c_void_p]),
+    'asac_policy_step_fused_loaded_offline': (C.c_int, [C.POINTER(MlpDesc), C.c_void_p, C.c_int64, C.POINTER(MlpDesc),
+                                                        C.c_void_p, C.c_int64, C.c_void_p, C.c_int64, C.c_int64, C.c_void_p,
+                                                        C.c_void_p, C.c_void_p, C.c_void_p, C.c_void_p, C.c_int64,
+                                                        C.c_void_p, C.c_void_p, C.c_void_p, C.c_void_p, C.c_int,
+                                                        C.c_void_p]),
     'asac_mlp_backward_policy_q': (C.c_int, [C.POINTER(MlpJob), C.c_void_p, C.c_void_p, C.c_int, C.c_void_p, C.c_void_p]),
     'asac_mlp_backward_policy_sample': (C.c_int, [C.POINTER(MlpJob), C.c_void_p, C.c_void_p, C.c_int, C.c_void_p,
                                                   C.c_void_p, C.c_void_p, C.c_int, C.c_void_p]),
@@ -1308,6 +1325,32 @@
                                                  _stream()), 'asac_mlp_backward_qloss_return')
 
 
+def policy_forward_save_floats(N: int) -> int:
+    return int(load().asac_policy_forward_save_floats(int(N)))
+
+
+def mlp_backward_qloss_return_rider_ok(job: MlpJob, ret: VtraceArgs, pi_job, save) -> bool:
+    return bool(load().asac_mlp_backward_qloss_return_rider_ok(C.byref(job), C.byref(ret),
+                                                               C.byref(pi_job) if pi_job is not None else None, _p(save)))
+
+
+def _mlp_backward_qloss_return_rider(job: MlpJob, target_q, ret: VtraceArgs, weights, clip_eps, loss_out, grad_params,
+                                     workspace, reduce_mode, pi_job: MlpJob, save, grad_x0=None):
+    global _last_work
+    _last_work = _pass_flops(job, backward=True) + _pass_flops(pi_job)
+    E, N = job.E, job.N
+    assert target_q.is_contiguous() and target_q.numel() == E * N
+    assert grad_x0 is None or (grad_x0.is_contiguous() and grad_x0.numel() == E * N * job.desc.contents.in0)
+    assert save.dtype == torch.float32 and save.is_contiguous() and save.numel() >= policy_forward_save_floats(pi_job.N)
+    _check(load().asac_mlp_backward_qloss_return_rider(C.byref(job), _p(target_q), C.byref(ret), _p(weights),
+                                                       float(clip_eps), _p(loss_out), _p(grad_x0), _p(grad_params),
+                                                       _p(workspace), int(reduce_mode), C.byref(pi_job), _p(save),
+                                                       _stream()), 'asac_mlp_backward_qloss_return_rider')
+
+
+mlp_backward_qloss_return_rider = _profiled(_mlp_backward_qloss_return_rider, 'asac_mlp_backward_qloss_return')
+
+
 @_profiled
 def mlp_backward_policy_q(job: MlpJob, q_table, subset, E_sample, grad_x1):
     global _last_work
@@ -1416,6 +1459,50 @@
 
 
 _policy_step_fused_plain = _profiled(_policy_step_fused, 'asac_policy_step_fused')
+
+
+def policy_step_fused_loaded_ok(q_desc, q_params, q_member_stride, pi_desc, pi_params, pi_member_stride, N, saved) -> bool:
+    return bool(load().asac_policy_step_fused_loaded_ok(C.byref(q_desc), _p(q_params), q_member_stride, C.byref(pi_desc),
+                                                        _p(pi_params), pi_member_stride, N, _p(saved)))
+
+
+def _policy_step_fused_loaded(q_desc, q_params, q_member_stride, pi_desc, pi_params, pi_member_stride, x, N, action, eps,
+                              log_alpha, saved, q_out, pi_grad_params, workspace, reduce_mode, subset=None, offline=None):
+    global _last_work
+    _last_work = (mlp_flops(q_desc, 2, N, backward=True, param_grads=False)
+                  + mlp_flops(pi_desc, 1, N, backward=True, param_grads=True))
+    p0, rs0, _ = _rows_view(x)
+    A = pi_desc.head_cols[0]
+    assert eps.is_contiguous() and eps.numel() == N * A
+    assert action is not None and action.is_contiguous() and action.numel() == N * A
+    assert saved.dtype == torch.float32 and saved.is_contiguous() and saved.numel() >= policy_forward_save_floats(N)
+    assert q_out is None or (q_out.is_contiguous() and q_out.numel() % N == 0 and q_out.numel() >= 2 * N)
+    assert subset is None or (subset.dtype == torch.int32 and subset.numel() == 2)
+    if offline is not None:
+        po, rso = _offline_view(offline, N, A)
+        _check(load().asac_policy_step_fused_loaded_offline(C.byref(q_desc), _p(q_params), q_member_stride,
+                                                            C.byref(pi_desc), _p(pi_params), pi_member_stride, p0, rs0, N,
+                                                            _p(action), _p(eps), _p(log_alpha), _p(subset), po, rso,
+                                                            _p(saved), _p(q_out), _p(pi_grad_params), _p(workspace),
+                                                            int(reduce_mode), _stream()),
+               'asac_policy_step_fused_loaded_offline')
+        return
+    _check(load().asac_policy_step_fused_loaded(C.byref(q_desc), _p(q_params), q_member_stride, C.byref(pi_desc),
+                                                _p(pi_params), pi_member_stride, p0, rs0, N, _p(action), _p(eps),
+                                                _p(log_alpha), _p(subset), _p(saved), _p(q_out), _p(pi_grad_params),
+                                                _p(workspace), int(reduce_mode), _stream()),
+           'asac_policy_step_fused_loaded')
+
+
+_policy_step_fused_loaded_plain = _profiled(_policy_step_fused_loaded, 'asac_policy_step_fused')
+_policy_step_fused_loaded_offline = _profiled(_policy_step_fused_loaded, 'asac_policy_step_fused_offline')
+
+
+def policy_step_fused_loaded(q_desc, q_params, q_member_stride, pi_desc, pi_params, pi_member_stride, x, N, action, eps,
+                             log_alpha, saved, q_out, pi_grad_params, workspace, reduce_mode, subset=None, offline=None):
+    fn = _policy_step_fused_loaded_plain if offline is None else _policy_step_fused_loaded_offline
+    return fn(q_desc, q_params, q_member_stride, pi_desc, pi_params, pi_member_stride, x, N, action, eps, log_alpha, saved,
+              q_out, pi_grad_params, workspace, reduce_mode, subset, offline)
 
 
 @_profiled
diff --git a/include/asac_hip.h b/include/asac_hip.h
--- a/include/asac_hip.h
+++ b/include/asac_hip.h
@@ -345,6 +345,14 @@
                                    const float* weights, float clip_eps, float* loss_out, float* grad_x0, float* grad_params,
                                    float* workspace, int reduce_mode, void* stream);
 
+int64_t asac_policy_forward_save_floats(int64_t N);
+int asac_mlp_backward_qloss_return_rider_ok(const asac_mlp_job_t* job, const asac_vtrace_args_t* ret,
+                                            const asac_mlp_job_t* pi_job, const float* save);
+int asac_mlp_backward_qloss_return_rider(const asac_mlp_job_t* job, const float* target_q, const asac_vtrace_args_t* ret,
+                                         const float* weights, float clip_eps, float* loss_out, float* grad_x0,
+                                         float* grad_params, float* workspace, int reduce_mode, const asac_mlp_job_t* pi_job,
+                                         float* save, void* stream);
+
 int asac_mlp_backward_policy_q(const asac_mlp_job_t* job, const float* q_table, const int32_t* subset, int E_sample,
                                float* grad_x1, void* stream);
 
@@ -362,6 +370,21 @@
                                    const float* log_alpha, const int32_t* subset, const float* off_action,
                                    int64_t off_row_stride, float* q_out, float* a_tanh_out, float* logp_out, float* ls_out,
                                    float* pi_grad_params, float* workspace, int reduce_mode, void* stream);
+
+int asac_policy_step_fused_loaded_ok(const asac_mlp_desc_t* q_desc, const float* q_params, int64_t q_member_stride,
+                                     const asac_mlp_desc_t* pi_desc, const float* pi_params, int64_t pi_member_stride, int64_t N,
+                                     const float* saved);
+int asac_policy_step_fused_loaded(const asac_mlp_desc_t* q_desc, const float* q_params, int64_t q_member_stride,
+                                  const asac_mlp_desc_t* pi_desc, const float* pi_params, int64_t pi_member_stride,
+                                  const float* x, int64_t x_row_stride, int64_t N, const float* action, const float* eps,
+                                  const float* log_alpha, const int32_t* subset, const float* saved, float* q_out,
+                                  float* pi_grad_params, float* workspace, int reduce_mode, void* stream);
+int asac_policy_step_fused_loaded_offline(const asac_mlp_desc_t* q_desc, const float* q_params, int64_t q_member_stride,
+                                          const asac_mlp_desc_t* pi_desc, const float* pi_params, int64_t pi_member_stride,
+                                          const float* x, int64_t x_row_stride, int64_t N, const float* action,
+                                          const float* eps, const float* log_alpha, const int32_t* subset,
+                                          const float* off_action, int64_t off_row_stride, const float* saved, float* q_out,
+                                          float* pi_grad_params, float* workspace, int reduce_mode, void* stream);
 
 int asac_mlp_backward_policy_sample(const asac_mlp_job_t* job, const float* eps, const float* grad_a, int grad_a_members,
                                     const float* log_alpha, float* grad_params, float* workspace, int reduce_mode,
```

Result: faster. 12890 train_steps/s, median of 6 (+2.2%).
